# rpng/ov_plane

Hardware: AMD Instinct MI355X
Metric: MSCKF+plane update-step features/sec at 30 clones (higher is better)
Workload: dtype f64

## Files before the change

ov_plane_amd/csrc/k_chol2.h:

```cpp
#pragma once
#include <hip/hip_runtime.h>

namespace ovp {

struct Chol2Job {
  const double* A;
  int n, ld;
  int add_identity;
  int mode;
  const int* sel;
  int sel_xor;
  size_t sel_stride;
  const double* brow;
  int* flag;
  const double* floor_scale;
  double piv_floor;
  double* Lpack;
  double* Ldense;
  int ldo;
  double* z_out;
  double* y_out;
  double* piv_out;
  double* Dinv_out;
  const int* skip_cond;
  long long* stamps;
  int dbg;
  int split_h;
  double* xbuf;
  unsigned* xflag;
  unsigned xseq;
  int flip;
  double* boost;
  int boost_n;
  double boost_rel;
};

struct PlaneSolve {
  double* scal;
  unsigned* range_done;
  unsigned seq;
  double thr;
  int rows_live, rows_u, n_involved;
  int force;
  double noise_scale;
  double tol_strict, tol_loose;
  double* res_out;
  double* xzz;
  double* xy;
  unsigned* xsync;
  const double* L0;
  int ld0;
  int n_full;
  double* dx_out;
  double* dx_last;
  int* cur;
  const int* feat_list;
  int n_feat_local;
  unsigned char* feat_used;
  double *clone_R, *clone_p;
  const int* clone_id;
  int n_clones;
  double* cal;
  int calib_id, intr_id;
  double* cp;
  const int* plane_sid;
  int n_planes;
  int n_slam;
  const int* slam_id;
  double* slam_p;
  int emit, seq_plane;
  double *Lpack, *Dinv;
  int* cond;
};

}

extern "C" {
int ovp_chol2_max_n(void);
int ovp_chol2_stamps_compiled(void);
hipError_t ovp_launch_max_diag(const double* A, int n, int ld, double* out, hipStream_t stream);
hipError_t ovp_launch_chol2_packed(const double* A, double* Dinv, double* Lpack, int n, int ld, int* flag, int add_identity,
                                   const int* cond, hipStream_t stream);
hipError_t ovp_launch_chol2(const ovp::Chol2Job* j0, const ovp::Chol2Job* j1, const ovp::PlaneSolve* ps, hipStream_t stream);
}
```

ov_plane_amd/csrc/k_chol2.hip:

```cpp
#include "k_tile_body.h"
#include "k_dpp.h"
#include "k_chol2.h"
#include <cstring>

namespace ovp {

static constexpr int C2_TS = 18;
static constexpr int C2_TSZ = 16 * C2_TS;
static constexpr int C2_WAVES = 12;
static constexpr int C2_EW = 4;
static constexpr int C2_TW = C2_WAVES - C2_EW;

typedef double dbl2_t __attribute__((ext_vector_type(2)));

template <bool HAS_FLOOR, bool WRITE_PIV, bool WRITE_D>
__device__ __forceinline__ bool fused_elim16(double (&d)[16], double (&p)[16], dbl2_t* __restrict__ pvw, const double floor,
                                             dbl2_t* __restrict__ pw, dbl2_t* __restrict__ dw, const int r) {
  double piv = bcast_row<0>(d[0]), piv_prev = 0.0;
  sfor<16>([&](auto cc) {
    constexpr int c = decltype(cc)::value;
    double y0 = __builtin_amdgcn_rsq(piv);
    if constexpr (HAS_FLOOR) y0 = (piv >= floor) ? y0 : 0.0;
    const double hy = (0.5 * piv) * y0;
    const double ly = d[c] * y0, py = p[c] * y0;
    const double e = fma(-hy, y0, 0.5);
    const double l = fma(ly, e, ly);
    const double q = fma(py, e, py);
    double nl;
    asm("v_fma_f64 %0, -%1, %2, -%1\n\ts_nop 1" : "=v"(nl) : "v"(ly), "v"(e));
    d[c] = l;
    p[c] = q;
    if constexpr (WRITE_PIV && (c & 1) == 1) pvw[c >> 1] = dbl2_t{piv_prev, piv};
    piv_prev = piv;
    if constexpr (c + 1 < 16) {
      fmac_bcast<c + 1>(d[c + 1], nl, l);
      piv = bcast_row<c + 1>(d[c + 1]);
      fmac_bcast<c + 1>(p[c + 1], nl, q);
      sfor<14 - c>([&](auto jc) {
        constexpr int j = c + 2 + decltype(jc)::value;
        fmac_bcast<j>(d[j], nl, l);
        fmac_bcast<j>(p[j], nl, q);
      });
    }
    if constexpr ((c & 1) == 1) pw[c >> 1] = dbl2_t{p[c - 1], p[c]};
    if constexpr (WRITE_D && (c & 1) == 1) dw[c >> 1] = dbl2_t{(c - 1 <= r) ? d[c - 1] : 0.0, (c <= r) ? d[c] : 0.0};
  });
  return HAS_FLOOR ? false : !(piv > 0.0);
}

__device__ __forceinline__ double4_t c2_mfma_xyT(const double* X, const double* Y, double4_t acc, int off) {
  const dbl2_t* xp = reinterpret_cast<const dbl2_t*>(reinterpret_cast<const char*>(X) + off);
  const dbl2_t* yp = reinterpret_cast<const dbl2_t*>(reinterpret_cast<const char*>(Y) + off);
  dbl2_t x0 = xp[0], y0 = yp[0], x1 = xp[1], y1 = yp[1];
  asm volatile("" : "+v"(x0), "+v"(y0), "+v"(x1), "+v"(y1));
  acc = __builtin_amdgcn_mfma_f64_16x16x4f64(x0[0], y0[0], acc, 0, 0, 1);
  acc = __builtin_amdgcn_mfma_f64_16x16x4f64(x0[1], y0[1], acc, 0, 0, 1);
  acc = __builtin_amdgcn_mfma_f64_16x16x4f64(x1[0], y1[0], acc, 0, 0, 1);
  acc = __builtin_amdgcn_mfma_f64_16x16x4f64(x1[1], y1[1], acc, 0, 0, 1);
  return acc;
}

template <int NH>
__device__ __forceinline__ void c2_last_update(double* Dbuf, double* Dupd, double* Lim, const double* pbp, int k, int i0, int g, int r,
                                               bool skip) {
  const double* Pk = pbp + k * C2_TSZ;
  const dbl2_t* yp = reinterpret_cast<const dbl2_t*>(Pk + r * C2_TS + 4 * g);
  const dbl2_t y0 = yp[0], y1 = yp[1];
  double4_t acc[NH + 1];
  dbl2_t x0[NH + 1], x1[NH + 1];
#pragma unroll
  for (int t = 0; t < NH; ++t) {
    const double* im = Lim + (i0 + C2_EW * t) * C2_TSZ;
#pragma unroll
    for (int v = 0; v < 4; ++v) acc[t][v] = im[(g + 4 * v) * C2_TS + r];
    const dbl2_t* xp = reinterpret_cast<const dbl2_t*>(pbp + (i0 + C2_EW * t) * C2_TSZ + r * C2_TS + 4 * g);
    x0[t] = xp[0];
    x1[t] = xp[1];
  }
#pragma unroll
  for (int v = 0; v < 4; ++v) acc[NH][v] = Dbuf[(g + 4 * v) * C2_TS + r];
  x0[NH] = y0;
  x1[NH] = y1;
  if (!skip) {
    constexpr int NS = NH <= 1 ? NH + 1 : 1;
    constexpr int S0 = NH + 1 - NS;
    double4_t acc2[NS];
#pragma unroll
    for (int t = 0; t < NS; ++t) acc2[t] = double4_t{0.0, 0.0, 0.0, 0.0};
#pragma unroll
    for (int t = 0; t <= NH; ++t) acc[t] = __builtin_amdgcn_mfma_f64_16x16x4f64(x0[t][0], y0[0], acc[t], 0, 0, 1);
#pragma unroll
    for (int t = 0; t < NS; ++t) acc2[t] = __builtin_amdgcn_mfma_f64_16x16x4f64(x1[S0 + t][0], y1[0], acc2[t], 0, 0, 1);
#pragma unroll
    for (int t = 0; t <= NH; ++t) acc[t] = __builtin_amdgcn_mfma_f64_16x16x4f64(x0[t][1], y0[1], acc[t], 0, 0, 1);
#pragma unroll
    for (int t = 0; t < NS; ++t) acc2[t] = __builtin_amdgcn_mfma_f64_16x16x4f64(x1[S0 + t][1], y1[1], acc2[t], 0, 0, 1);
#pragma unroll
    for (int t = 0; t < S0; ++t) acc[t] = __builtin_amdgcn_mfma_f64_16x16x4f64(x1[t][0], y1[0], acc[t], 0, 0, 1);
#pragma unroll
    for (int t = 0; t < S0; ++t) acc[t] = __builtin_amdgcn_mfma_f64_16x16x4f64(x1[t][1], y1[1], acc[t], 0, 0, 1);
#pragma unroll
    for (int t = 0; t < NS; ++t) acc[S0 + t] = acc[S0 + t] + acc2[t];
  }
#pragma unroll
  for (int t = 0; t < NH; ++t) {
    double* im = Lim + (i0 + C2_EW * t) * C2_TSZ;
#pragma unroll
    for (int v = 0; v < 4; ++v) im[(g + 4 * v) * C2_TS + r] = acc[t][v];
  }
#pragma unroll
  for (int v = 0; v < 4; ++v) Dupd[(g + 4 * v) * C2_TS + r] = acc[NH][v];
}

__device__ __forceinline__ void c2_store_through_sys(double* p, dbl2_t v) {
  asm volatile("global_store_dwordx4 %0, %1, off sc0 sc1\n\ts_nop 1" ::"v"(p), "v"(v) : "memory");
}
__device__ __forceinline__ void c2_load2_through_sys(const double* p0, const double* p1, dbl2_t& v0, dbl2_t& v1) {
  asm volatile(
      "global_load_dwordx4 %0, %2, off sc0 sc1\n\t"
      "global_load_dwordx4 %1, %3, off sc0 sc1\n\t"
      "s_waitcnt vmcnt(0)"
      : "=&v"(v0), "=&v"(v1)
      : "v"(p0), "v"(p1)
      : "memory");
}

#define C2_WSYNC()                                           \
  do {                                                       \
    __builtin_amdgcn_fence(__ATOMIC_RELEASE, "workgroup");   \
    __builtin_amdgcn_wave_barrier();                         \
    __builtin_amdgcn_fence(__ATOMIC_ACQUIRE, "workgroup");   \
  } while (0)

static constexpr int C2_SPIN_LIMIT = 1 << 22;
__device__ __forceinline__ void c2_wait_ge(int* ctr, int target, int* tmo) {
  int spins = 0;
  while (__hip_atomic_load(ctr, __ATOMIC_RELAXED, __HIP_MEMORY_SCOPE_WORKGROUP) < target) {
    asm volatile("s_nop 7");
    if (__builtin_expect(++spins > C2_SPIN_LIMIT, 0)) {
      __hip_atomic_store(tmo, 1, __ATOMIC_RELAXED, __HIP_MEMORY_SCOPE_WORKGROUP);
      break;
    }
  }
  __builtin_amdgcn_fence(__ATOMIC_ACQUIRE, "workgroup");
}
__device__ __forceinline__ void c2_signal(int* ctr, int lane) {
  const unsigned a = (unsigned)(size_t)(__attribute__((address_space(3))) int*)ctr;
  asm volatile("" ::: "memory");
  if (lane == 0) asm volatile("ds_add_u32 %0, %1" ::"v"(a), "v"(1) : "memory");
  asm volatile("" ::: "memory");
}

template <int MAXSLOT, class F>
__device__ __forceinline__ void slot_range(int lo, int hi, F&& f) {
  if (lo > hi) return;
#define C2_CASE(S)                                                        \
  case S:                                                                 \
    if constexpr (S < MAXSLOT) f(std::integral_constant<int, S>{});       \
    if (hi <= S) break;                                                   \
    [[fallthrough]];
  switch (lo) {
    C2_CASE(0) C2_CASE(1) C2_CASE(2) C2_CASE(3) C2_CASE(4) C2_CASE(5) C2_CASE(6) C2_CASE(7) C2_CASE(8) C2_CASE(9) C2_CASE(10)
// ... 513 lines not shown
    for (int e = lane; e < C2_TSZ; e += 64) SD[(nt - 1) * C2_TSZ + e] = 0.0;
  if (wave == 2 || wave == 3)
    for (int e = (wave - 2) * 64 + lane; e < nt * C2_TW * 16; e += 128) SL[e] = 0.0;
  BS_STAMP(nt, 4);
  __syncthreads();
  BS_STAMP(nt, 5);
  if constexpr (ROLE == 0) {
  if (wave == 0) {
    const int r = lc;
    double y = k_hi < nt ? S.ybuf[16 * k_hi + r] : 0.0;
    double sd[16], di[16];
    auto load_sd = [&](int k) {
      const double* sblk = SD + (k >= 0 ? k : 0) * C2_TSZ + r;
#pragma unroll
      for (int c = 0; c < 16; ++c) sd[c] = sblk[c * C2_TS];
    };
    auto load_di = [&](int k) {
      const double* dblk = S.Dsave + (k >= 0 ? k : 0) * C2_TSZ + r;
#pragma unroll
      for (int c = 0; c < 16; ++c) di[c] = dblk[c * C2_TS];
    };
    load_sd(k_hi - 1);
    load_di(k_hi - 1);
    for (int k = k_hi - 1; k >= k_lo; --k) {
      BS_STAMP(k, 4);
      static_assert(C2_TW == 8, "eight partial vectors");
      const int kc = k <= nt - 3 ? k : 0;
      const double* sl = SL + ((size_t)kc * C2_TW) * 16 + r;
      int got = __hip_atomic_load(cnt_s + kc, __ATOMIC_RELAXED, __HIP_MEMORY_SCOPE_WORKGROUP);
      asm volatile("" ::: "memory");
      double p0 = sl[0], p1 = sl[16], p2 = sl[32], p3 = sl[48], p4 = sl[64], p5 = sl[80], p6 = sl[96], p7 = sl[112];
      double v = S.zbuf[16 * k + r];
      double t0 = 0.0, t1 = 0.0, t2 = 0.0, t3 = 0.0;
      fmac_bcast_nop<0>(t0, y, sd[0]);
      fmac_bcast_nop<1>(t1, y, sd[1]);
      fmac_bcast_nop<2>(t2, y, sd[2]);
      fmac_bcast_nop<3>(t3, y, sd[3]);
      fmac_bcast<4>(t0, y, sd[4]);
      fmac_bcast<5>(t1, y, sd[5]);
      fmac_bcast<6>(t2, y, sd[6]);
      fmac_bcast<7>(t3, y, sd[7]);
      fmac_bcast<8>(t0, y, sd[8]);
      fmac_bcast<9>(t1, y, sd[9]);
      fmac_bcast<10>(t2, y, sd[10]);
      fmac_bcast<11>(t3, y, sd[11]);
      fmac_bcast<12>(t0, y, sd[12]);
      fmac_bcast<13>(t1, y, sd[13]);
      fmac_bcast<14>(t2, y, sd[14]);
      fmac_bcast<15>(t3, y, sd[15]);
      double tsum = (t0 + t1) + (t2 + t3);
      asm volatile("" : "+v"(tsum));
      load_sd(k - 1);
      BS_STAMP(k, 5);
      if (k <= nt - 3) {
        const int need = (nt - k - 2 < C2_TW) ? nt - k - 2 : C2_TW;
        int spins = 0;
        while (got < need) {
          asm volatile("s_nop 7");
          if (__builtin_expect(++spins > C2_SPIN_LIMIT, 0)) {
            __hip_atomic_store(S.cnt + 6, 1, __ATOMIC_RELAXED, __HIP_MEMORY_SCOPE_WORKGROUP);
            break;
          }
          got = __hip_atomic_load(cnt_s + k, __ATOMIC_RELAXED, __HIP_MEMORY_SCOPE_WORKGROUP);
          asm volatile("" ::: "memory");
          p0 = sl[0], p1 = sl[16], p2 = sl[32], p3 = sl[48], p4 = sl[64], p5 = sl[80], p6 = sl[96], p7 = sl[112];
          asm volatile("" : "+v"(p0), "+v"(p1), "+v"(p2), "+v"(p3), "+v"(p4), "+v"(p5), "+v"(p6), "+v"(p7));
        }
        BS_STAMP(k, 6);
        v -= ((p0 + p1) + (p2 + p3)) + ((p4 + p5) + (p6 + p7));
      }
      v -= tsum;
      if (16 * k + r >= n) v = 0.0;
      double y0 = 0.0, y1 = 0.0, y2 = 0.0, y3 = 0.0;
      fmac_bcast_nop<0>(y0, v, di[0]);
      fmac_bcast_nop<1>(y1, v, di[1]);
      fmac_bcast_nop<2>(y2, v, di[2]);
      fmac_bcast_nop<3>(y3, v, di[3]);
      fmac_bcast<4>(y0, v, di[4]);
      fmac_bcast<5>(y1, v, di[5]);
      fmac_bcast<6>(y2, v, di[6]);
      fmac_bcast<7>(y3, v, di[7]);
      fmac_bcast<8>(y0, v, di[8]);
      fmac_bcast<9>(y1, v, di[9]);
      fmac_bcast<10>(y2, v, di[10]);
      fmac_bcast<11>(y3, v, di[11]);
      fmac_bcast<12>(y0, v, di[12]);
      fmac_bcast<13>(y1, v, di[13]);
      fmac_bcast<14>(y2, v, di[14]);
      fmac_bcast<15>(y3, v, di[15]);
      y = (y0 + y1) + (y2 + y3);
      if (16 * k + r >= n) y = 0.0;
      if (lane < 16) S.ybuf[16 * k + r] = y;
      c2_signal(cnt_y, lane);
      load_di(k - 1);
      BS_STAMP(k, 7);
    }
  }
  } else {
    const int tw = wave - C2_EW;
    int cur = nt;
    int pub = nt - k_hi;
    double part = 0.0;
    bool any = false;
    auto flush_to = [&](int jnew) {
      if (any && cur <= nt - 3) {
        const double pv = rows_sum_f64(part);
        if (lane < 16) SL[((size_t)cur * C2_TW + tw) * 16 + lane] = pv;
        c2_signal(cnt_s + cur, lane);
      }
      cur = jnew;
      part = 0.0;
      any = false;
    };
    sfor<MAXSLOT>([&](auto sc) {
      constexpr int s = MAXSLOT - 1 - decltype(sc)::value;
      const int i = ti[s], j = tj[s];
      if (i >= 0 && i < nt) {
        if (j != cur) flush_to(j);
        if (i >= j + 2) {
          if (pub < nt - i) {
            c2_wait_ge(cnt_y, nt - i, S.cnt + 6);
            pub = nt - i;
          }
#pragma unroll
          for (int v = 0; v < 4; ++v) part = fma(tile[s][v], S.ybuf[16 * i + lr + 4 * v], part);
          any = true;
        }
      }
    });
    flush_to(-1);
  }
  __syncthreads();
}

__device__ __forceinline__ void c2_pack_tile(double* __restrict__ Lpack, const double4_t& t, int i, int j, int n, int lr, int lc,
                                             int n_layout = 0) {
  const int ntn = ((n_layout > 0 ? n_layout : n) + 15) >> 4;
  const int tidx = j * ntn - (j * (j - 1)) / 2 + (i - j);
  double* pk = Lpack + (size_t)tidx * 256;
#pragma unroll
  for (int v = 0; v < 4; ++v) {
    const int row = lr + 4 * v, col = lc;
    const int gr = 16 * i + row, gc = 16 * j + col;
    double x = t[v];
    if (gr >= n || gc >= n) x = (gr == gc) ? 1.0 : 0.0;
    if (i == j && col > row) x = 0.0;
    pk[col * 16 + row] = x;
  }
}

static constexpr size_t C2_PS_KERNARG_OFFSET = (2 * sizeof(Chol2Job) + alignof(PlaneSolve) - 1) / alignof(PlaneSolve) * alignof(PlaneSolve);
static_assert(sizeof(Chol2Job) % alignof(Chol2Job) == 0 && alignof(Chol2Job) == 8 && alignof(PlaneSolve) == 8, "kernel-argument layout");

struct Chol2Shared {
  int bad, ok;
  double zz;
};

template <int MAXSLOT, int ROLE, bool SPLIT>
__device__ __forceinline__ void chol2_body(const Chol2Job& J0_, const PlaneSolve& ps, double* lds, Chol2Shared& sh, const int joff) {
  typedef const Chol2Job __attribute__((address_space(4))) Chol2JobK;
  typedef const char __attribute__((address_space(4))) KernargByte;
  Chol2JobK& Jf = *(Chol2JobK*)((KernargByte*)__builtin_amdgcn_kernarg_segment_ptr() + joff);
  const int n = Jf.n;
  const int nb = Jf.brow ? n + 1 : n;
  const int nt = (nb + 15) >> 4;
  const Chol2Lds S = chol2_carve(lds, nt);
  constexpr int NS = ROLE == 1 ? MAXSLOT : 1;
  if (Jf.skip_cond && Jf.skip_cond[0] != 0 && Jf.skip_cond[0] == Jf.skip_cond[1]) return;
  double4_t tile[NS];
  int ti[NS], tj[NS];
  int bad = 0;
  int& sh_bad = sh.bad;
  int& sh_ok = sh.ok;
  double& sh_zz = sh.zz;
  if (threadIdx.x == 0) sh_bad = 0;
  const int part = (SPLIT && Jf.mode == 1 && Jf.split_h > 0) ? (blockIdx.x == 2 ? 1 : 0) : -1;
  const int c_lo = part == 1 ? Jf.split_h : 0, c_hi = part == 0 ? Jf.split_h : nt;
#if C2_STAMPS_ON
  Chol2Job Jl = J0_;
  if (part == 1 && Jl.stamps) Jl.stamps += 16 * 32;
  const Chol2Job& J = Jl;
  chol2_factor<NS, ROLE, SPLIT, Chol2Job>(J, S, tile, ti, tj, bad, c_lo, c_hi);
#else
  chol2_factor<NS, ROLE, SPLIT, Chol2JobK>(Jf, S, tile, ti, tj, bad, c_lo, c_hi);
#endif
  const int tid = threadIdx.x, lane = tid & 63;
  const int wave = __builtin_amdgcn_readfirstlane(tid >> 6);
  const int lr = lane >> 4, lc = lane & 15;
  if (bad && lane == 0) atomicOr(&sh_bad, 1);
  __syncthreads();
  if (tid == 0 && S.cnt[6]) atomicOr(&sh_bad, 2);
  __syncthreads();
  bad = sh_bad;
  typedef const PlaneSolve __attribute__((address_space(4))) PlaneSolveK;
  PlaneSolveK* pk = (PlaneSolveK*)((KernargByte*)__builtin_amdgcn_kernarg_segment_ptr() + C2_PS_KERNARG_OFFSET);
  Chol2JobK* jk = (Chol2JobK*)((KernargByte*)__builtin_amdgcn_kernarg_segment_ptr() + joff);
  asm volatile("" : "+s"(pk), "+s"(jk));
  PlaneSolveK& pq = *pk;
  Chol2JobK& jq = *jk;
  if (bad && tid == 0 && jq.flag) atomicOr(jq.flag, bad);

  if (jq.mode == 0) {
    if (jq.z_out)
      for (int i = tid; i < n; i += C2_WAVES * 64) jq.z_out[i] = S.zbuf[i];
    if (jq.y_out) {
      chol2_backsolve<NS, ROLE>(S, n, (n + 15) >> 4, tile, ti, tj, jq.stamps);
      for (int i = tid; i < n; i += C2_WAVES * 64) jq.y_out[i] = S.ybuf[i];
    }
    if constexpr (ROLE == 1) {
    sfor<MAXSLOT>([&](auto sc) {
      constexpr int s = decltype(sc)::value;
      if (ti[s] >= 0) {
        if (jq.Ldense) {
#pragma unroll
          for (int v = 0; v < 4; ++v) {
            const int rr = 16 * ti[s] + lr + 4 * v, cc = 16 * tj[s] + lc;
            if (rr < nb && cc < nb) {
              const int ro = jq.flip ? n - 1 - rr : rr, rz = jq.flip ? n - 1 - cc : cc;
              jq.Ldense[(size_t)ro * jq.ldo + cc] = (cc <= rr) ? tile[s][v] : 0.0;
              if (ti[s] != tj[s]) jq.Ldense[(size_t)rz * jq.ldo + rr] = 0.0;
            }
          }
        }
        if (jq.Lpack && 16 * ti[s] < n && 16 * tj[s] < n) c2_pack_tile(jq.Lpack, tile[s], ti[s], tj[s], n, lr, lc);
      }
    });
    }
    if (jq.piv_out)
      for (int i = tid; i < n; i += C2_WAVES * 64) jq.piv_out[i] = S.pivs[i];
    if (jq.Dinv_out) {
      const int ntn = (n + 15) >> 4;
      if constexpr (ROLE == 0)
        if (!jq.y_out) c2_invert_diag_blocks(S, 0, ntn, wave, lr, lc);
      __syncthreads();
      if constexpr (ROLE == 0) {
        for (int e = tid; e < ntn * 256; e += C2_EW * 64) {
          const int k = e >> 8, i = (e >> 4) & 15, c = e & 15;
          const int gr = 16 * k + i, gc = 16 * k + c;
          jq.Dinv_out[e] = (gr < n && gc < n) ? S.Dsave[k * C2_TSZ + i * C2_TS + c] : (i == c ? 1.0 : 0.0);
        }
      }
    }
    return;
  }

  if (jq.mode == 2) {
    if (wave == 0) {
      double pr = 0.0;
      for (int i = lane; i < n; i += 64) pr = fma(S.zbuf[i], S.zbuf[i], pr);
      pr = wave_sum(pr);
      int first = 0x7fffffff, n_strict = 0;
      for (int i = lane; i < pq.n_involved; i += 64) {
        if (S.pivs[i] < pq.tol_strict) {
          ++n_strict;
          first = i < first ? i : first;
        }
      }
#pragma unroll
      for (int m = 32; m >= 1; m >>= 1) {
        n_strict += __shfl_xor(n_strict, m);
        const int o = __shfl_xor(first, m);
        first = o < first ? o : first;
      }
      int n_loose = 0;
      for (int i = lane; i < pq.n_involved; i += 64) {
        const double pv = S.pivs[i];
        if (i > first && !(pv < pq.tol_strict) && pv < pq.tol_loose) ++n_loose;
      }
#pragma unroll
      for (int m = 32; m >= 1; m >>= 1) n_loose += __shfl_xor(n_loose, m);
      if (lane == 0) {
        const int ndeg = n_strict + n_loose;
        pq.scal[1] = pr;
        pq.scal[2] = (double)ndeg;
        __threadfence();
        __hip_atomic_store(pq.range_done, pq.seq, __ATOMIC_RELEASE, __HIP_MEMORY_SCOPE_AGENT);
      }
    }
    return;
  }

#define M1_STAMP(i) C2_STAMP(nt + 1, i)
  M1_STAMP(0);
  if (wave == 0) {
    double zz = 0.0;
    for (int i = lane; i < n; i += 64) zz = fma(S.zbuf[i], S.zbuf[i], zz);
    zz = wave_sum(zz);
    if (lane == 0 && part == 0) {
      pq.xzz[0] = zz;
      pq.xzz[1] = (double)bad;
      __hip_atomic_store(pq.xsync, pq.seq, __ATOMIC_RELEASE, __HIP_MEMORY_SCOPE_AGENT);
      int spins = 0;
      unsigned v = 0u;
      bool timed_out = false;
      while (((v = __hip_atomic_load(pq.xsync + 1, __ATOMIC_ACQUIRE, __HIP_MEMORY_SCOPE_AGENT)) >> 1) != (pq.seq & 0x7fffffffu)) {
        __builtin_amdgcn_s_sleep(2);
        if (++spins > (1 << 19)) {
          timed_out = true;
          break;
        }
      }
      if (timed_out && jq.flag) atomicOr(jq.flag, 2);
      sh_zz = zz;
      sh_ok = (!timed_out && (v & 1u)) ? 1 : 0;
    } else if (lane == 0) {
      int spins = 0;
      bool timed_out = false;
      if (part == 1) {
        while (__hip_atomic_load(pq.xsync, __ATOMIC_ACQUIRE, __HIP_MEMORY_SCOPE_AGENT) != pq.seq) {
          __builtin_amdgcn_s_sleep(1);
          if (++spins > (1 << 19)) {
            timed_out = true;
            break;
          }
        }
        zz += pq.xzz[0];
        bad |= (int)pq.xzz[1];
        spins = 0;
      }
      while (__hip_atomic_load(pq.range_done, __ATOMIC_ACQUIRE, __HIP_MEMORY_SCOPE_AGENT) != pq.seq) {
        __builtin_amdgcn_s_sleep(2);
        if (++spins > (1 << 18)) {
          timed_out = true;
          break;
        }
      }
      if (timed_out && jq.flag) atomicOr(jq.flag, 2);
      const double rr = pq.scal[0], pr = pq.scal[1], ndeg = pq.scal[2];
      const double rank = (double)pq.n_involved - ndeg;
      const double noise_rows = fmax((double)pq.rows_u - rank, 0.0);
      const double denom = (double)pq.rows_live - rank;
      const double frac = denom > 0.5 ? fmin(noise_rows / denom, 1.0) : 1.0;
      const double chi2 = (pr - zz) + pq.noise_scale * frac * fmax(rr - pr, 0.0);
      const int upstream = jq.flag ? __hip_atomic_load(jq.flag, __ATOMIC_RELAXED, __HIP_MEMORY_SCOPE_AGENT) : 0;
      const bool fact_ok = (bad == 0) && !timed_out && upstream == 0;
      const bool ok = fact_ok && (pq.force == 0 ? false : (pq.force == 1 ? true : (chi2 <= pq.thr)));
      pq.res_out[0] = chi2;
      pq.res_out[1] = ok ? 1.0 : 0.0;
      pq.res_out[2] = ndeg;
      pq.res_out[3] = pr;
      sh_zz = zz;
      sh_ok = ok ? 1 : 0;
      if (part == 1 && !ok)
        __hip_atomic_store(pq.xsync + 1, (pq.seq & 0x7fffffffu) << 1, __ATOMIC_RELEASE, __HIP_MEMORY_SCOPE_AGENT);
    }
  }
  __syncthreads();
  if (!sh_ok) return;
  M1_STAMP(1);

  const int ntn = (n + 15) >> 4;
  const int h_bs = part >= 0 ? (jq.split_h < ntn ? jq.split_h : ntn) : 0;
  if (part == 0)
    for (int i = 16 * h_bs + tid; i < 16 * ntn; i += C2_WAVES * 64) S.ybuf[i] = pq.xy[i];
  chol2_backsolve<NS, ROLE>(S, n, ntn, tile, ti, tj, nullptr, part == 0 ? h_bs : ntn, part == 1 ? h_bs : 0);
  M1_STAMP(2);
  if (part == 1) {
    for (int i = 16 * h_bs + tid; i < 16 * ntn; i += C2_WAVES * 64) pq.xy[i] = S.ybuf[i];
    __syncthreads();
    if (tid == 0) {
      const bool fine = S.cnt[6] == 0;
      if (!fine) {
        if (jq.flag) atomicOr(jq.flag, 2);
        pq.res_out[1] = 0.0;
      }
      __hip_atomic_store(pq.xsync + 1, ((pq.seq & 0x7fffffffu) << 1) | (fine ? 1u : 0u), __ATOMIC_RELEASE, __HIP_MEMORY_SCOPE_AGENT);
    }
    if (pq.cond && pq.emit && S.cnt[6] == 0) {
      if constexpr (ROLE == 1) {
        sfor<MAXSLOT>([&](auto sc) {
          constexpr int s = decltype(sc)::value;
          if (ti[s] >= 0 && 16 * ti[s] < n && 16 * tj[s] < n) c2_pack_tile(pq.Lpack, tile[s], ti[s], tj[s], n, lr, lc, pq.n_full);
        });
      } else {
        for (int e = 256 * h_bs + tid; e < ntn * 256; e += C2_EW * 64) {
          const int k = e >> 8, i = (e >> 4) & 15, c = e & 15;
          const int gr = 16 * k + i, gc = 16 * k + c;
          pq.Dinv[e] = (gr < n && gc < n) ? S.Dsave[k * C2_TSZ + i * C2_TS + c] : (i == c ? 1.0 : 0.0);
        }
      }
    }
    return;
  }
  const int nfull = pq.n_full > n ? pq.n_full : n;
  double* dxs = nfull > n ? S.PB : S.zbuf;
  __syncthreads();
  if (S.cnt[6]) {
    if (tid == 0) {
      if (jq.flag) atomicOr(jq.flag, 2);
      pq.res_out[1] = 0.0;
    }
    return;
  }
  {
    const int wv = tid >> 6, ln = tid & 63;
    dbl2_t yp[3];
#pragma unroll
    for (int k = 0; k < 3; ++k) {
      const int c0 = 2 * (ln + 64 * k);
      yp[k][0] = c0 < n ? S.ybuf[c0] : 0.0;
      yp[k][1] = c0 + 1 < n ? S.ybuf[c0 + 1] : 0.0;
    }
    auto batch = [&](auto jlo_c, auto cnt_c, auto k_c) {
      constexpr int JLO = decltype(jlo_c)::value, CNT = decltype(cnt_c)::value, K = decltype(k_c)::value;
      constexpr int NP = CNT <= 2 ? 2 : (CNT <= 4 ? 4 : (CNT <= 8 ? 8 : 16));
      if (12 * JLO >= nfull) return;
      dbl2_t v[CNT][K];
#pragma unroll
      for (int j = 0; j < CNT; ++j) {
        const int row = wv + 12 * (JLO + j);
        const int lastc = row < n ? row : n - 1;
        const int npair = (lastc + 2) >> 1;
        const dbl2_t* lrow = reinterpret_cast<const dbl2_t*>(pq.L0 + (size_t)row * pq.ld0);
#pragma unroll
        for (int k = 0; k < K; ++k) {
          const int q = ln + 64 * k;
          v[j][k] = (row < nfull && q < npair) ? lrow[q] : dbl2_t{0.0, 0.0};
        }
      }
      double part[NP];
#pragma unroll
      for (int j = 0; j < NP; ++j) part[j] = 0.0;
#pragma unroll
      for (int j = 0; j < CNT; ++j) {
        const int row = wv + 12 * (JLO + j);
        const int lastc = row < n ? row : n - 1;
        double sa = 0.0;
#pragma unroll
        for (int k = 0; k < K; ++k) {
          const int c0 = 2 * (ln + 64 * k);
          sa = fma(v[j][k][0], yp[k][0], sa);
          sa = fma(c0 + 1 <= lastc ? v[j][k][1] : 0.0, yp[k][1], sa);
        }
        part[j] = sa;
      }
      const double tot = wave_transpose_reduce<NP>(part);
      const int jo = ln / (64 / NP);
      const int row = wv + 12 * (JLO + jo);
      if ((ln % (64 / NP)) == 0 && jo < CNT && row < nfull) dxs[row] = tot;
    };
    batch(std::integral_constant<int, 0>{}, std::integral_constant<int, 8>{}, std::integral_constant<int, 1>{});
    batch(std::integral_constant<int, 8>{}, std::integral_constant<int, 2>{}, std::integral_constant<int, 1>{});
    batch(std::integral_constant<int, 10>{}, std::integral_constant<int, 4>{}, std::integral_constant<int, 2>{});
    batch(std::integral_constant<int, 14>{}, std::integral_constant<int, 4>{}, std::integral_constant<int, 2>{});
    batch(std::integral_constant<int, 18>{}, std::integral_constant<int, 3>{}, std::integral_constant<int, 2>{});
    batch(std::integral_constant<int, 21>{}, std::integral_constant<int, 3>{}, std::integral_constant<int, 3>{});
  }
  __syncthreads();
  M1_STAMP(3);
  for (int i = tid; i < nfull; i += C2_WAVES * 64) {
    pq.dx_out[i] = dxs[i];
    pq.dx_last[i] = dxs[i];
  }
  if (tid == 0) *pq.cur ^= 1;
  for (int i = tid; i < pq.n_feat_local; i += C2_WAVES * 64) pq.feat_used[pq.feat_list[i]] = 1;
  auto rot_update = [&](double* R, const double* dth) {
    double qx = 0.5 * dth[0], qy = 0.5 * dth[1], qz = 0.5 * dth[2], qw = 1.0;
    const double nn = 1.0 / sqrt(qx * qx + qy * qy + qz * qz + qw * qw);
    qx *= nn;
    qy *= nn;
    qz *= nn;
    qw *= nn;
    const double a = 2.0 * qw * qw - 1.0;
    double D[9];
    D[0] = a + 2.0 * qx * qx;
    D[1] = 2.0 * qw * qz + 2.0 * qx * qy;
    D[2] = -2.0 * qw * qy + 2.0 * qx * qz;
    D[3] = -2.0 * qw * qz + 2.0 * qy * qx;
    D[4] = a + 2.0 * qy * qy;
    D[5] = 2.0 * qw * qx + 2.0 * qy * qz;
    D[6] = 2.0 * qw * qy + 2.0 * qz * qx;
    D[7] = -2.0 * qw * qx + 2.0 * qz * qy;
    D[8] = a + 2.0 * qz * qz;
    double O[9];
    for (int i = 0; i < 3; ++i)
      for (int j = 0; j < 3; ++j) O[3 * i + j] = D[3 * i] * R[j] + D[3 * i + 1] * R[3 + j] + D[3 * i + 2] * R[6 + j];
    for (int i = 0; i < 9; ++i) R[i] = O[i];
  };
  if (tid < pq.n_clones) {
    const int id = pq.clone_id[tid];
    rot_update(pq.clone_R + 9 * tid, dxs + id);
    for (int k = 0; k < 3; ++k) pq.clone_p[3 * tid + k] += dxs[id + 3 + k];
  } else if (tid == pq.n_clones) {
    if (pq.calib_id >= 0) {
      rot_update(pq.cal, dxs + pq.calib_id);
      for (int k = 0; k < 3; ++k) pq.cal[9 + k] += dxs[pq.calib_id + 3 + k];
    }
    if (pq.intr_id >= 0)
      for (int k = 0; k < 8; ++k) pq.cal[12 + k] += dxs[pq.intr_id + k];
  } else if (tid > pq.n_clones && tid <= pq.n_clones + pq.n_planes) {
    const int pl = tid - pq.n_clones - 1;
    if (pq.plane_sid[pl] >= 0)
      for (int k = 0; k < 3; ++k) pq.cp[3 * pl + k] += dxs[pq.plane_sid[pl] + k];
  }
  for (int q = tid; q < pq.n_slam; q += C2_WAVES * 64)
    for (int k = 0; k < 3; ++k) pq.slam_p[3 * q + k] += dxs[pq.slam_id[q] + k];
  M1_STAMP(4);
  if (pq.cond) {
    if (tid == 0) pq.cond[1] = pq.seq_plane;
    if (pq.emit) {
      if constexpr (ROLE == 1) {
        sfor<MAXSLOT>([&](auto sc) {
          constexpr int s = decltype(sc)::value;
          if (ti[s] >= 0 && 16 * ti[s] < n && 16 * tj[s] < n) c2_pack_tile(pq.Lpack, tile[s], ti[s], tj[s], n, lr, lc, pq.n_full);
        });
      } else {
        for (int e = tid; e < (part == 0 ? h_bs : ntn) * 256; e += C2_EW * 64) {
          const int k = e >> 8, i = (e >> 4) & 15, c = e & 15;
          const int gr = 16 * k + i, gc = 16 * k + c;
          pq.Dinv[e] = (gr < n && gc < n) ? S.Dsave[k * C2_TSZ + i * C2_TS + c] : (i == c ? 1.0 : 0.0);
        }
        if (tid == 0) pq.cond[0] = pq.seq_plane;
      }
    }
  }
}

template <int MAXSLOT, bool SPLIT>
__global__ __launch_bounds__(C2_WAVES * 64) void k_chol2(const Chol2Job J0, const Chol2Job J1, const PlaneSolve ps) {
  extern __shared__ __attribute__((aligned(16))) double lds[];
  __shared__ Chol2Shared sh;
  const Chol2Job& J = blockIdx.x == 1 ? J1 : J0;
  const int wave = __builtin_amdgcn_readfirstlane((int)threadIdx.x >> 6);
  const int joff = blockIdx.x == 1 ? (int)sizeof(Chol2Job) : 0;
  if (wave < C2_EW) chol2_body<MAXSLOT, 0, SPLIT>(J, ps, lds, sh, joff);
  else chol2_body<MAXSLOT, 1, SPLIT>(J, ps, lds, sh, joff);
}

__global__ __launch_bounds__(256) void k_max_diag(const double* __restrict__ A, int n, int ld, double* __restrict__ out) {
  __shared__ double red[256];
  double m = 0.0;
  for (int i = threadIdx.x; i < n; i += 256) m = fmax(m, A[(size_t)i * ld + i]);
  red[threadIdx.x] = m;
  __syncthreads();
  for (int s = 128; s > 0; s >>= 1) {
    if ((int)threadIdx.x < s) red[threadIdx.x] = fmax(red[threadIdx.x], red[threadIdx.x + s]);
    __syncthreads();
  }
  if (threadIdx.x == 0) out[0] = red[0];
}

}

extern "C" {

hipError_t ovp_launch_max_diag(const double* A, int n, int ld, double* out, hipStream_t stream) {
  hipLaunchKernelGGL(ovp::k_max_diag, dim3(1), dim3(256), 0, stream, A, n, ld, out);
  return hipGetLastError();
}

int ovp_chol2_max_n(void) { return 16 * 18 - 1; }

hipError_t ovp_launch_chol2_packed(const double* A, double* Dinv, double* Lpack, int n, int ld, int* flag, int add_identity,
                                   const int* cond, hipStream_t stream) {
  ovp::Chol2Job j;
  memset(&j, 0, sizeof(j));
  j.A = A;
  j.n = n;
  j.ld = ld;
  j.add_identity = add_identity;
  j.mode = 0;
  j.flag = flag;
  j.Lpack = Lpack;
  j.Dinv_out = Dinv;
  j.skip_cond = cond;
  return ovp_launch_chol2(&j, nullptr, nullptr, stream);
}

int ovp_chol2_stamps_compiled(void) { return C2_STAMPS_ON; }

hipError_t ovp_launch_chol2(const ovp::Chol2Job* j0, const ovp::Chol2Job* j1, const ovp::PlaneSolve* ps, hipStream_t stream) {
  using namespace ovp;
  auto ntof = [](const Chol2Job* j) { return ((j->brow ? j->n + 1 : j->n) + 15) / 16; };
  int nt = ntof(j0);
  int tiles = nt * (nt + 1) / 2;
  if (j0->split_h > 0) {
    const int h = j0->split_h;
    if (!j1 || !ps || j0->mode != 1 || h >= nt || !j0->xbuf || !j0->xflag || !ps->xzz || !ps->xy || !ps->xsync) return hipErrorInvalidValue;
    const int ta = h * nt - (h * (h - 1)) / 2;
    tiles = ta > tiles - ta ? ta : tiles - ta;
  }
  if (j1) {
    const int nt1 = ntof(j1);
    if (nt1 * (nt1 + 1) / 2 > tiles) tiles = nt1 * (nt1 + 1) / 2;
    if (nt1 > nt) nt = nt1;
  }
  const int slots = (tiles + C2_TW - 1) / C2_TW;
  const size_t shmem = (size_t)chol2_lds_doubles(nt) * sizeof(double);
  Chol2Job dummy = *j0;
  PlaneSolve psd = PlaneSolve();
  const Chol2Job& b = j1 ? *j1 : dummy;
  const PlaneSolve& p = ps ? *ps : psd;
  const dim3 grid(j0->split_h > 0 ? 3 : (j1 ? 2 : 1)), block(C2_WAVES * 64);
  static unsigned long long attr_mask = 0;
  if (ovp_lds_attr_needed(&attr_mask)) {
    (void)hipFuncSetAttribute((const void*)k_chol2<10, false>, hipFuncAttributeMaxDynamicSharedMemorySize, 160 * 1024);
    (void)hipFuncSetAttribute((const void*)k_chol2<15, false>, hipFuncAttributeMaxDynamicSharedMemorySize, 160 * 1024);
    (void)hipFuncSetAttribute((const void*)k_chol2<17, false>, hipFuncAttributeMaxDynamicSharedMemorySize, 160 * 1024);
    (void)hipFuncSetAttribute((const void*)k_chol2<20, false>, hipFuncAttributeMaxDynamicSharedMemorySize, 160 * 1024);
    (void)hipFuncSetAttribute((const void*)k_chol2<22, false>, hipFuncAttributeMaxDynamicSharedMemorySize, 160 * 1024);
    (void)hipFuncSetAttribute((const void*)k_chol2<13, true>, hipFuncAttributeMaxDynamicSharedMemorySize, 160 * 1024);
    (void)hipFuncSetAttribute((const void*)k_chol2<16, true>, hipFuncAttributeMaxDynamicSharedMemorySize, 160 * 1024);
    (void)hipFuncSetAttribute((const void*)k_chol2<22, true>, hipFuncAttributeMaxDynamicSharedMemorySize, 160 * 1024);
    (void)hipGetLastError();
    ovp_lds_attr_done(&attr_mask);
  }
  if (j0->split_h > 0) {
    if (slots <= 13)
      hipLaunchKernelGGL((k_chol2<13, true>), grid, block, shmem, stream, *j0, b, p);
    else if (slots <= 16)
      hipLaunchKernelGGL((k_chol2<16, true>), grid, block, shmem, stream, *j0, b, p);
    else if (slots <= 22)
      hipLaunchKernelGGL((k_chol2<22, true>), grid, block, shmem, stream, *j0, b, p);
    else
      return hipErrorInvalidValue;
    return hipGetLastError();
  }
  if (slots <= 10)
    hipLaunchKernelGGL((k_chol2<10, false>), grid, block, shmem, stream, *j0, b, p);
  else if (slots <= 15)
    hipLaunchKernelGGL((k_chol2<15, false>), grid, block, shmem, stream, *j0, b, p);
  else if (slots <= 17)
    hipLaunchKernelGGL((k_chol2<17, false>), grid, block, shmem, stream, *j0, b, p);
  else if (slots <= 20)
    hipLaunchKernelGGL((k_chol2<20, false>), grid, block, shmem, stream, *j0, b, p);
  else if (slots <= 22)
    hipLaunchKernelGGL((k_chol2<22, false>), grid, block, shmem, stream, *j0, b, p);
  else
    return hipErrorInvalidValue;
  return hipGetLastError();
}
}
```

ov_plane_amd/csrc/ovp_api_ctx.hip:

```cpp
#include "ovp_ctx.h"

static double gammap_reg(double a, double x) {
  if (x <= 0) return 0.0;
  const double gln = lgamma(a);
  if (x < a + 1.0) {
    double ap = a, sum = 1.0 / a, del = sum;
    for (int n = 0; n < 100000; ++n) {
      ap += 1.0;
      del *= x / ap;
      sum += del;
      if (fabs(del) < fabs(sum) * 1e-17) break;
    }
    return sum * exp(-x + a * log(x) - gln);
  }
  double b = x + 1.0 - a, c = 1.0 / 1e-300, d = 1.0 / b, h = d;
  for (int i = 1; i < 100000; ++i) {
    const double an = -i * (i - a);
    b += 2.0;
    d = an * d + b;
    if (fabs(d) < 1e-300) d = 1e-300;
    c = b + an / c;
    if (fabs(c) < 1e-300) c = 1e-300;
    d = 1.0 / d;
    const double del = d * c;
// ... 32 lines not shown
  switch (code) {
    case 0: return "ok";
    case OVP_E_ARG: return "bad argument";
    case OVP_E_CAPACITY: return "capacity exceeded";
    case OVP_E_NOTSPD: return "matrix not positive definite";
    case OVP_E_NEGDIAG: return "negative covariance diagonal";
    case OVP_E_NODEVICE: return "no usable HIP device";
    case OVP_E_STATE: return "call order violated";
    case OVP_E_TIMEOUT: return "device-side hand-over timed out (workgroups of the plane solve not co-resident)";
    case OVP_E_RCCL: return "RCCL not loadable or a collective call failed";
    case OVP_E_PEER: return "sharded update: the build of another rank failed (errors are collective)";
    default: return code > 0 ? hipGetErrorString((hipError_t)code) : "unknown";
  }
}


extern "C" int ovp_ctx_create(int device, int n_state_max, int n_clones_max, int n_feats_max, void* stream,
                              ovp_ctx** out) {
  if (!out || n_state_max < 1 || n_clones_max < 1 || n_clones_max > OVP_MAX_CLONES || n_feats_max < 1) return OVP_E_ARG;
  int ndev = 0;
  if (hipGetDeviceCount(&ndev) != hipSuccess || ndev <= device) return OVP_E_NODEVICE;
  HIPCHK(hipSetDevice(device));
  hipDeviceProp_t prop;
  HIPCHK(hipGetDeviceProperties(&prop, device));
  if (strncmp(prop.gcnArchName, "gfx950", 6) != 0) return OVP_E_NODEVICE;
  ovp_ctx* c = new ovp_ctx();
  c->device = device;
  if (stream) {
    c->stream = (hipStream_t)stream;
  } else {
    HIPCHK(hipStreamCreateWithFlags(&c->stream, hipStreamNonBlocking));
    c->own_stream = true;
  }
  HIPCHK(hipStreamCreateWithFlags(&c->stream2, hipStreamNonBlocking));
  HIPCHK(hipEventCreateWithFlags(&c->ev_fork, hipEventDisableTiming));
  HIPCHK(hipEventCreateWithFlags(&c->ev_join, hipEventDisableTiming));
  for (int i = 0; i < 6; ++i) HIPCHK(hipEventCreate(&c->ev_t[i]));
  HIPCHK(hipEventCreate(&c->ev_k0));
  HIPCHK(hipEventCreate(&c->ev_k1));
  c->n_max = n_state_max;
  c->c_max = n_clones_max;
  c->f_max = n_feats_max;
  c->ld = round_up(n_state_max, 16);
  c->ldg = round_up(n_state_max + 4, 16);
  if (c->ldg > OVP_LDG_CAP) return OVP_E_CAPACITY;
  const size_t nn = (size_t)(c->n_max + 1) * c->ld;
  HIPCHK(dalloc(&c->P, nn));
  HIPCHK(dalloc(&c->P_tmp, nn));
  HIPCHK(dalloc(&c->Ab, nn + 8));
  HIPCHK(dalloc(&c->L, nn));
  HIPCHK(dalloc(&c->W1, nn));
  HIPCHK(dalloc(&c->T, nn));
  HIPCHK(dalloc(&c->Lt, nn));
  HIPCHK(dalloc(&c->Y, nn));
  c->res_bytes = 16 + sizeof(double) * ((size_t)c->n_max + n_feats_max) + (size_t)n_feats_max;
  HIPCHK(hipMalloc((void**)&c->res_block, c->res_bytes));
  HIPCHK(hipMemset(c->res_block, 0, c->res_bytes));
  c->flags = (int*)c->res_block;
  c->dx = (double*)((char*)c->res_block + 16);
  c->chi2 = c->dx + c->n_max;
  c->accept = (unsigned char*)(c->chi2 + n_feats_max);
  {
    auto al = [](size_t v) { return (v + 63) & ~(size_t)63; };
    size_t o = 0;
    c->so_R = o;
    o = al(o + sizeof(double) * 9 * n_clones_max);
    c->so_Rf = o;
    o = al(o + sizeof(double) * 9 * n_clones_max);
    c->so_p = o;
    o = al(o + sizeof(double) * 3 * n_clones_max);
    c->so_pf = o;
    o = al(o + sizeof(double) * 3 * n_clones_max);
    c->so_cal = o;
    o = al(o + sizeof(double) * 32);
    c->so_id = o;
    o = al(o + sizeof(int) * n_clones_max);
    c->so_cm = o;
    o = al(o + sizeof(ovp::ColMap) * c->n_max);
    c->state_bytes = o;
    HIPCHK(hipMalloc(&c->state_block, o));
    HIPCHK(hipMemset(c->state_block, 0, o));
    HIPCHK(hipHostMalloc(&c->h_state_stage, o, hipHostMallocDefault));
    char* b = (char*)c->state_block;
    c->clone_R = (double*)(b + c->so_R);
    c->clone_R_fej = (double*)(b + c->so_Rf);
    c->clone_p = (double*)(b + c->so_p);
    c->clone_p_fej = (double*)(b + c->so_pf);
    c->cal = (double*)(b + c->so_cal);
    c->clone_id = (int*)(b + c->so_id);
    c->colmap = (ovp::ColMap*)(b + c->so_cm);
    HIPCHK(hipEventCreateWithFlags(&c->ev_state, hipEventDisableTiming));
    HIPCHK(hipEventCreateWithFlags(&c->ev_batch, hipEventDisableTiming));
  }
  HIPCHK(dalloc(&c->chi2_table, (size_t)OVP_CHI2_TABLE + 1));
  {
    const size_t F = (size_t)n_feats_max, M = OVP_MAX_MEAS;
    c->batch_cap = sizeof(double) * 3 * F + sizeof(int) * F + sizeof(int) * F * M + sizeof(float) * 2 * F * M + 256;
    HIPCHK(hipMalloc(&c->batch_block, c->batch_cap));
    HIPCHK(hipHostMalloc(&c->h_batch_stage, c->batch_cap, hipHostMallocDefault));
    c->p_FinG = (double*)c->batch_block;
  }
  HIPCHK(dalloc(&c->G, (size_t)3 * n_feats_max * c->ldg));
  HIPCHK(dalloc(&c->Bscr, (size_t)n_feats_max * OVP_BSCR));
  HIPCHK(dalloc(&c->rec, (size_t)n_clones_max * n_feats_max * 2 * 21));
  c->rows_per_chunk = 128;
  c->n_chunks = (2 * n_feats_max + c->rows_per_chunk - 1) / c->rows_per_chunk;
  HIPCHK(dalloc(&c->gramS, (size_t)n_clones_max * c->n_chunks * OVP_GRAM_ELEMS));
  HIPCHK(dalloc(&c->gramR, (size_t)n_clones_max * OVP_GRAM_ELEMS));
  HIPCHK(dalloc(&c->Dinv, (size_t)(c->ld / 16 + 1) * 256));
  {
    const size_t ntm = (size_t)c->ld / 16 + 1;
    HIPCHK(dalloc(&c->Ltp, ntm * (ntm + 1) / 2 * 256));
  }
  c->n_split = (3 * n_feats_max + 63) / 64;
  if (c->n_split < 1) c->n_split = 1;
  if (c->n_split > 64) c->n_split = 64;
  {
    const int nt = c->ldg / 16;
    HIPCHK(dalloc(&c->part, (size_t)(c->n_split + 1) * (nt * (nt + 1) / 2) * 256));
  }
  HIPCHK(dalloc(&c->idbuf, (size_t)4 * c->n_max + 64));
  c->small_cap = (size_t)4 * c->n_max * 64 + (size_t)c->n_max * c->n_max;
  HIPCHK(dalloc(&c->smallbuf, c->small_cap));
  HIPCHK(hipMalloc((void**)&c->ticket, 16));
  HIPCHK(hipMemset(c->ticket, 0, 16));
  HIPCHK(hipHostMalloc((void**)&c->h_res_block, c->res_bytes + 64, hipHostMallocMapped));
  memset(c->h_res_block, 0, c->res_bytes + 64);
  HIPCHK(hipHostGetDevicePointer(&c->h_res_block_dev, c->h_res_block, 0));
  HIPCHK(hipHostMalloc((void**)&c->h_slot, sizeof(int) * (size_t)(n_feats_max + 16), hipHostMallocMapped));
  HIPCHK(hipHostGetDevicePointer((void**)&c->d_slot, c->h_slot, 0));
  c->h_seq = (volatile unsigned*)((char*)c->h_res_block + ((c->res_bytes + 15) & ~(size_t)15));
  c->h_flags = (int*)c->h_res_block;
  c->h_dx = (double*)((char*)c->h_res_block + 16);
  c->h_chi2 = c->h_dx + c->n_max;
  c->h_accept = (unsigned char*)(c->h_chi2 + n_feats_max);
  {
    std::vector<double> tab(OVP_CHI2_TABLE + 1, 0.0);
    for (int k = 1; k <= OVP_CHI2_TABLE; ++k) tab[k] = ovp_chi2_quantile_095(k);
    HIPCHK(hipMemcpy(c->chi2_table, tab.data(), sizeof(double) * tab.size(), hipMemcpyHostToDevice));
  }
  memset(&c->fp, 0, sizeof(c->fp));
  *out = c;
  return 0;
}

extern "C" int ovp_ctx_destroy(ovp_ctx* c) {
  if (!c) return OVP_E_ARG;
  hipSetDevice(c->device);
  hipStreamSynchronize(c->stream);
  hipStreamSynchronize(c->stream2);
  void* dev[] = {c->P, c->P_tmp, c->Ab, c->L, c->W1, c->T, c->Lt, c->Y, c->res_block, c->ticket, c->uvn, c->tri_ok, c->state_block, c->batch_block,
                 c->chi2_table, c->G, c->Bscr, c->rec, c->gramS, c->gramR, c->Dinv, c->Ltp, c->part, c->idbuf, c->smallbuf, c->Hd, c->Acc,
                 c->bcc, c->resd, c->pl_slam_i, c->pl_slam_d, c->sub_ids, c->sub_buf, c->pl_Tbuf, c->pl_crow, c->pl_dxlast,
                 c->pl_cur, c->pl_perm, c->pl_range_done, c->pl_used, c->pl_dstage, c->pl_xbuf, c->pl_xy, c->pl_xflag, c->pl_Asum,
                 c->pl_U, c->pl_sub_tab, c->Lkeep, c->slam_res, c->slam_hscr, c->dinit_buf, c->boost, c->boost_vec,
                 c->gen_cal, c->gen_buf, c->pl_gen_dev};
  for (void* p : dev)
    if (p) hipFree(p);
  if (c->h_res_block) hipHostFree(c->h_res_block);
  if (c->h_slot) hipHostFree(c->h_slot);
  if (c->h_state_stage) hipHostFree(c->h_state_stage);
  if (c->h_batch_stage) hipHostFree(c->h_batch_stage);
  if (c->ev_state) hipEventDestroy(c->ev_state);
  if (c->ev_batch) hipEventDestroy(c->ev_batch);
  if (c->pl_hstage) hipHostFree(c->pl_hstage);
  if (c->pl_hres) hipHostFree(c->pl_hres);
  if (c->pl_sub_htab) hipHostFree(c->pl_sub_htab);
  if (c->ev_subtab) hipEventDestroy(c->ev_subtab);
  for (hipEvent_t e : c->pl_ev) hipEventDestroy(e);
  for (hipEvent_t e : c->pl_ev_loop) hipEventDestroy(e);
  if (c->io_h) hipHostFree(c->io_h);
  if (c->io_d) hipFree(c->io_d);
  hipEventDestroy(c->ev_fork);
  hipEventDestroy(c->ev_join);
  for (int i = 0; i < 6; ++i) hipEventDestroy(c->ev_t[i]);
  hipEventDestroy(c->ev_k0);
  hipEventDestroy(c->ev_k1);
  hipStreamDestroy(c->stream2);
  if (c->own_stream) hipStreamDestroy(c->stream);
  delete c;
  return 0;
}

extern "C" int ovp_sync(ovp_ctx* c) {
  if (!c) return OVP_E_ARG;
  HIPCHK(hipStreamSynchronize(c->stream));
  return 0;
}

extern "C" int ovp_ctx_stream(ovp_ctx* c, void** stream) {
  if (!c || !stream) return OVP_E_ARG;
  *stream = (void*)c->stream;
  return 0;
}

extern "C" int ovp_cov_size(ovp_ctx* c) { return c ? c->n : OVP_E_ARG; }

extern "C" int ovp_io_arena(ovp_ctx* c, size_t bytes, void** host, void** dev);

extern "C" int ovp_cov_upload(ovp_ctx* c, const double* P_host, int n, int ld) {
  drop_kept_factor(c);
  if (!c || !P_host || n < 1 || ld < n) return OVP_E_ARG;
  if (n > c->n_max) return OVP_E_CAPACITY;
  void *ah = nullptr, *ad = nullptr;
  const size_t bytes = sizeof(double) * (size_t)n * c->ld;
  {
    const int rca = ovp_io_arena(c, bytes, &ah, &ad);
    if (rca) return rca;
  }
  for (int i = 0; i < n; ++i) {
    memcpy((double*)ah + (size_t)i * c->ld, P_host + (size_t)i * ld, sizeof(double) * n);
    if (c->ld > n) memset((double*)ah + (size_t)i * c->ld + n, 0, sizeof(double) * (c->ld - n));
  }
  HIPCHK(hipMemcpyAsync(c->P, ah, bytes, hipMemcpyHostToDevice, c->stream));
  HIPCHK(hipStreamSynchronize(c->stream));
  c->n = n;
  c->have_cov = true;
  return 0;
}
extern "C" int ovp_cov_set_device(ovp_ctx* c, const double* P_dev, int n, int ld) {
  drop_kept_factor(c);
  if (!c || !P_dev || n < 1 || ld < n) return OVP_E_ARG;
  if (n > c->n_max) return OVP_E_CAPACITY;
  HIPCHK(hipMemcpy2DAsync(c->P, sizeof(double) * c->ld, P_dev, sizeof(double) * ld, sizeof(double) * n, n,
                          hipMemcpyDeviceToDevice, c->stream));
  c->n = n;
  c->have_cov = true;
  return 0;
}
extern "C" int ovp_cov_download(ovp_ctx* c, double* P_host, int n, int ld) {
  if (!c || !P_host || n != c->n || ld < n) return OVP_E_ARG;
  void *ah = nullptr, *ad = nullptr;
  const size_t bytes = sizeof(double) * (size_t)n * c->ld;
  {
    const int rca = ovp_io_arena(c, bytes, &ah, &ad);
    if (rca) return rca;
  }
  HIPCHK(hipMemcpyAsync(ah, c->P, bytes, hipMemcpyDeviceToHost, c->stream));
  HIPCHK(hipStreamSynchronize(c->stream));
  for (int i = 0; i < n; ++i) memcpy(P_host + (size_t)i * ld, (const double*)ah + (size_t)i * c->ld, sizeof(double) * n);
  return 0;
}
extern "C" int ovp_cov_marginal(ovp_ctx* c, const int* ids, const int* sizes, int n_vars, double* out_host) {
  if (!c || !ids || !sizes || !out_host || n_vars < 1) return OVP_E_ARG;
  std::vector<int> cols;
  for (int i = 0; i < n_vars; ++i)
    for (int k = 0; k < sizes[i]; ++k) {
      if (ids[i] + k >= c->n || ids[i] < 0) return OVP_E_ARG;
      cols.push_back(ids[i] + k);
    }
  const int m = (int)cols.size();
  if (m > c->n_max || (size_t)m * m > c->small_cap) return OVP_E_CAPACITY;
  void *ah = nullptr, *ad = nullptr;
  const size_t o_out = ((sizeof(int) * (size_t)m + 63) / 64) * 64, bytes = o_out + sizeof(double) * (size_t)m * m;
  {
    const int rca = ovp_io_arena(c, bytes, &ah, &ad);
    if (rca) return rca;
  }
  memcpy(ah, cols.data(), sizeof(int) * m);
  HIPCHK(hipMemcpyAsync(ad, ah, sizeof(int) * m, hipMemcpyHostToDevice, c->stream));
  HIPCHK(ovp_launch_gather_marginal(c->P, c->ld, (const int*)ad, m, (double*)((char*)ad + o_out), c->stream));
  HIPCHK(hipMemcpyAsync((char*)ah + o_out, (char*)ad + o_out, sizeof(double) * (size_t)m * m, hipMemcpyDeviceToHost, c->stream));
  HIPCHK(hipStreamSynchronize(c->stream));
  memcpy(out_host, (char*)ah + o_out, sizeof(double) * (size_t)m * m);
  return 0;
}

void quat_2_rot(const double q[4], double R[9]) {
  const double x = q[0], y = q[1], z = q[2], w = q[3];
  const double a = 2.0 * w * w - 1.0;
  R[0] = a + 2.0 * x * x;
  R[1] = 2.0 * w * z + 2.0 * x * y;
  R[2] = -2.0 * w * y + 2.0 * x * z;
  R[3] = -2.0 * w * z + 2.0 * y * x;
  R[4] = a + 2.0 * y * y;
  R[5] = 2.0 * w * x + 2.0 * y * z;
  R[6] = 2.0 * w * y + 2.0 * z * x;
  R[7] = -2.0 * w * x + 2.0 * z * y;
  R[8] = a + 2.0 * z * z;
}

extern "C" int ovp_state_upload(ovp_ctx* c, const ovp_state_tables* st) {
  if (!c || !st || !st->clone_q || !st->clone_p || !st->clone_q_fej || !st->clone_p_fej || !st->clone_id) return OVP_E_ARG;
  if (st->n_clones < 1 || st->n_clones > c->c_max || st->n_state > c->n_max) return OVP_E_CAPACITY;
  const int C = st->n_clones;
  for (int i = 0; i < C; ++i)
    if (st->clone_id[i] < 0 || st->clone_id[i] + 6 > st->n_state) return OVP_E_ARG;
  HIPCHK(hipEventSynchronize(c->ev_state));
  char* h = (char*)c->h_state_stage;
  double* R = (double*)(h + c->so_R);
  double* Rf = (double*)(h + c->so_Rf);
  for (int i = 0; i < C; ++i) {
    quat_2_rot(st->clone_q + 4 * i, R + 9 * i);
    quat_2_rot(st->clone_q_fej + 4 * i, Rf + 9 * i);
  }
  memcpy(h + c->so_p, st->clone_p, sizeof(double) * 3 * C);
  memcpy(h + c->so_pf, st->clone_p_fej, sizeof(double) * 3 * C);
  memcpy(h + c->so_id, st->clone_id, sizeof(int) * C);
  {
    double* cal = (double*)(h + c->so_cal);
    quat_2_rot(st->calib_q, cal);
    memcpy(cal + 9, st->calib_p, sizeof(double) * 3);
    memcpy(cal + 12, st->intrinsics, sizeof(double) * 8);
  }
  ovp::ColMap* cm = (ovp::ColMap*)(h + c->so_cm);
  memset(cm, 0, sizeof(ovp::ColMap) * c->n_max);
  for (int i = 0; i < C; ++i)
// ... 192 lines not shown
extern "C" int ovp_cov_clone_jitter(ovp_ctx* c, double relative_inflation) {
  if (!c || !(relative_inflation >= 0.0) || relative_inflation > 1e-6) return OVP_E_ARG;
  c->clone_jitter = relative_inflation;
  return 0;
}

extern "C" int ovp_cov_marginalize(ovp_ctx* c, int id, int size) {
  drop_kept_factor(c);
  if (!c || size < 1 || id < 0) return OVP_E_ARG;
  if (!c->have_cov) return OVP_E_STATE;
  if (id + size > c->n) return OVP_E_ARG;
  HIPCHK(ovp_launch_cov_marginalize(c->P, c->P_tmp, c->ld, c->n, id, size, c->stream));
  double* t = c->P;
  c->P = c->P_tmp;
  c->P_tmp = t;
  c->n -= size;
  return 0;
}

extern "C" int ovp_cov_initialize_invertible(ovp_ctx* c, const double* H_R, int k, int cols, int ld, const int* col_ids,
                                             const double* H_Linv, const double* R) {
  drop_kept_factor(c);
  if (!c || !H_R || !col_ids || !H_Linv || !R || k < 1 || k > 6 || cols < 1 || ld < k) return OVP_E_ARG;
  if (!c->have_cov) return OVP_E_STATE;
  const int n = c->n;
  if (n + k > c->n_max) return OVP_E_CAPACITY;
  if (cols > c->n_max) return OVP_E_ARG;
  for (int j = 0; j < cols; ++j)
    if (col_ids[j] < 0 || col_ids[j] >= n) return OVP_E_ARG;
  std::vector<double> hr((size_t)k * cols), hi((size_t)k * k), rk((size_t)k * k);
  for (int i = 0; i < k; ++i)
    for (int a = 0; a < cols; ++a) hr[(size_t)i * cols + a] = H_R[(size_t)a * ld + i];
  for (int i = 0; i < k; ++i)
    for (int j = 0; j < k; ++j) {
      hi[(size_t)i * k + j] = H_Linv[(size_t)j * k + i];
      rk[(size_t)i * k + j] = R[(size_t)j * k + i];
    }
  double* dHR = c->smallbuf;
  double* dHi = dHR + (size_t)k * cols;
  double* dRk = dHi + 36;
  double* dMa = dRk + 36;
  if ((size_t)(dMa + (size_t)6 * n - c->smallbuf) > c->small_cap) return OVP_E_CAPACITY;
  HIPCHK(hipMemcpyAsync(dHR, hr.data(), sizeof(double) * hr.size(), hipMemcpyHostToDevice, c->stream));
  HIPCHK(hipMemcpyAsync(dHi, hi.data(), sizeof(double) * hi.size(), hipMemcpyHostToDevice, c->stream));
  HIPCHK(hipMemcpyAsync(dRk, rk.data(), sizeof(double) * rk.size(), hipMemcpyHostToDevice, c->stream));
  HIPCHK(hipMemcpyAsync(c->idbuf, col_ids, sizeof(int) * cols, hipMemcpyHostToDevice, c->stream));
  HIPCHK(ovp_launch_init_invertible(c->P, c->ld, n, c->idbuf, cols, dHR, k, dMa, dHi, dRk, c->stream));
  HIPCHK(hipStreamSynchronize(c->stream));
  c->n = n + k;
  return 0;
}

extern "C" int ovp_cov_augment_dt(ovp_ctx* c, int pose_id, int dt_id, const double dnc_dt[6]) {
  drop_kept_factor(c);
  if (!c || !dnc_dt) return OVP_E_ARG;
  if (!c->have_cov) return OVP_E_STATE;
  if (pose_id < 0 || pose_id + 6 > c->n || dt_id < 0 || dt_id >= c->n) return OVP_E_ARG;
  HIPCHK(ovp_launch_augment_dt(c->P, c->ld, c->n, pose_id, dt_id, dnc_dt, c->stream));
  return 0;
}

extern "C" int ovp_cov_initialize(ovp_ctx* c, const double* Hx_init, const double* H_up, int k, int rup, int cols, const int* col_ids,
                                  const double* H_Linv, const double* R_init, const double* res_up, double r_iso,
                                  double chi2_threshold, int do_update, int* accepted, double* chi2, double* dx_host) {
  drop_kept_factor(c);
  if (!c || !Hx_init || !col_ids || !H_Linv || !R_init || k < 1 || k > 6 || cols < 1 || rup < 0) return OVP_E_ARG;
  if (rup > 0 && (!H_up || !res_up || !(r_iso > 0.0))) return OVP_E_ARG;
  if (!c->have_cov) return OVP_E_STATE;
  const int n = c->n, n2 = n + k, ld = c->ld, m = k + rup;
  if (n2 > c->n_max || cols > c->n_max) return OVP_E_CAPACITY;
  if (rup > ovp_init_max_rows() || ovp_init_core_lds(k, rup, cols) > ovp_init_max_lds()) return OVP_E_CAPACITY;
  for (int j = 0; j < cols; ++j)
    if (col_ids[j] < 0 || col_ids[j] >= n) return OVP_E_ARG;
  hipStream_t s = c->stream;
  const bool upd = rup > 0 && do_update;
  const size_t oHt = 0, oHi = oHt + (size_t)cols * m, oRk = oHi + 36, oRes = oRk + 36, oId = oRes + rup + 8;
  const size_t bytes = oId * sizeof(double) + sizeof(int) * (size_t)cols + 64;
  const size_t res_doubles = 4 + (size_t)c->n_max + 8;
  int rc = plane2_buffers(c, 0, bytes, res_doubles * sizeof(double));
  if (rc) return rc;
  double* h = (double*)c->pl_hstage;
  double* d = (double*)c->pl_dstage;
  for (int a = 0; a < cols; ++a) {
    double* row = h + oHt + (size_t)a * m;
    for (int i = 0; i < k; ++i) row[i] = Hx_init[(size_t)a * k + i];
    for (int i = 0; i < rup; ++i) row[k + i] = H_up[(size_t)a * rup + i];
  }
  for (int i = 0; i < 36; ++i) h[oHi + i] = h[oRk + i] = 0.0;
  for (int i = 0; i < k; ++i)
    for (int j = 0; j < k; ++j) {
      h[oHi + (size_t)i * k + j] = H_Linv[(size_t)j * k + i];
      h[oRk + (size_t)i * k + j] = R_init[(size_t)j * k + i];
    }
  for (int i = 0; i < rup; ++i) h[oRes + i] = res_up[i];
  memcpy(h + oId, col_ids, sizeof(int) * cols);
  const int* did = (const int*)(d + oId);
  double* dres = c->smallbuf;
  double* dM = dres + res_doubles;
  double* dLi = dM + (size_t)n2 * m;
  double* dy = dLi + (size_t)rup * rup;
  if ((size_t)(dy + rup + 8 - c->smallbuf) > c->small_cap) return OVP_E_CAPACITY;
  HIPCHK(hipMemcpyAsync(c->pl_dstage, c->pl_hstage, bytes, hipMemcpyHostToDevice, s));
  HIPCHK(ovp_launch_init_m(c->P, ld, n, did, cols, d + oHt, m, dM, s));
  HIPCHK(ovp_launch_init_core(c->P, ld, n, did, cols, d + oHt, k, rup, dM, d + oHi, d + oRk, d + oRes, r_iso > 0.0 ? r_iso : 1.0,
                              chi2_threshold, dLi, dy, dres, s));
  double* hres = (double*)c->pl_hres;
  if (upd) {
    HIPCHK(ovp_launch_init_update(c->P, c->P_tmp, ld, n2, dM, m, k, rup, dLi, dy, dres, dres + 4, s));
  }
  {
    const int rf = ovp_fetch_to_hres(c, dres, sizeof(double) * (upd ? 4 + (size_t)n2 : 4), s);
    if (rf) return rf;
  }
  const bool ok = hres[1] > 0.5;
  if (accepted) *accepted = ok ? 1 : 0;
  if (chi2) *chi2 = hres[0];
  if (!ok) return 0;
  c->n = n2;
  if (upd) {
    double* t = c->P;
    c->P = c->P_tmp;
    c->P_tmp = t;
  }
  if (dx_host) {
    if (upd) memcpy(dx_host, hres + 4, sizeof(double) * n2);
    else memset(dx_host, 0, sizeof(double) * n2);
  }
  if (upd && hres[2] != 0.0) return OVP_E_NEGDIAG;
  return 0;
}

extern "C" long ovp_debug_read(ovp_ctx* c, const char* name, void* host, long max_bytes) {
  if (!c || !name || !host) return OVP_E_ARG;
  const size_t nn = (size_t)(c->n_max + 1) * c->ld * sizeof(double);
  const void* src = nullptr;
  size_t bytes = 0;
  if (!strcmp(name, "A") || !strcmp(name, "Ab")) { src = c->Ab; bytes = nn; }
  else if (!strcmp(name, "L")) { src = c->L; bytes = nn; }
  else if (!strcmp(name, "T")) { src = c->T; bytes = nn; }
  else if (!strcmp(name, "Lt")) { src = c->Lt; bytes = nn; }
  else if (!strcmp(name, "Y")) { src = c->Y; bytes = nn; }
  else if (!strcmp(name, "W1")) { src = c->W1; bytes = nn; }
  else if (!strcmp(name, "P")) { src = c->P; bytes = nn; }
  else if (!strcmp(name, "G")) { src = c->G; bytes = (size_t)3 * c->n_feats * c->ldg * sizeof(double); }
  else if (!strcmp(name, "rec")) { src = c->rec; bytes = (size_t)c->fp.n_clones * c->n_feats * 2 * 21 * sizeof(double); }
  else if (!strcmp(name, "plres")) { src = c->pl_res; bytes = (size_t)4 * c->pl_cap * sizeof(double); if (!src) return OVP_E_STATE; }
  else if (!strcmp(name, "An")) { src = c->pl_An; bytes = nn; if (!src) return OVP_E_STATE; }
  else if (!strcmp(name, "bn")) { src = c->pl_bn; bytes = (size_t)c->n_max * sizeof(double); if (!src) return OVP_E_STATE; }
  else if (!strcmp(name, "pl_hres_cap")) {
    if ((size_t)max_bytes < sizeof(size_t)) return OVP_E_ARG;
    memcpy(host, &c->pl_hres_cap, sizeof(size_t));
    return (long)sizeof(size_t);
  }
  else if (!strcmp(name, "cal")) { src = c->cal; bytes = 20 * sizeof(double); if (!src) return OVP_E_STATE; }
  else if (!strcmp(name, "gen_cal")) { src = c->gen_cal; bytes = (size_t)20 * c->gen_ncams * sizeof(double); if (!src) return OVP_E_STATE; }
  else if (!strcmp(name, "dinit_planes")) {
    if (!c->pl_dstage || c->dinit_nplanes < 1) return OVP_E_STATE;
    src = (const char*)c->pl_dstage + c->dinit_pltab_off;
    bytes = (size_t)8 * c->dinit_nplanes * sizeof(double);
  }
  else if (!strcmp(name, "chi2")) {
    hipStreamSynchronize(c->stream);
    bytes = (size_t)c->n_feats * sizeof(double);
    if ((long)bytes > max_bytes) bytes = (size_t)max_bytes;
    memcpy(host, c->h_chi2, bytes);
    return (int)bytes;
  }
  else if (!strncmp(name, "bench_chol", 10)) {
    ovp_dbg_tilechol_skip = atoi(name + 10);
    hipEvent_t e0, e1;
    hipEventCreate(&e0);
    hipEventCreate(&e1);
    for (int i = 0; i < 3; ++i) ovp_launch_tilechol(c->P, c->L, c->Dinv, c->Ltp, c->n, c->ld, c->flags + 3, 0, c->stream);
    hipEventRecord(e0, c->stream);
    for (int i = 0; i < 20; ++i) ovp_launch_tilechol(c->P, c->L, c->Dinv, c->Ltp, c->n, c->ld, c->flags + 3, 0, c->stream);
    hipEventRecord(e1, c->stream);
    hipEventSynchronize(e1);
    float ms = 0.f;
    hipEventElapsedTime(&ms, e0, e1);
    ovp_dbg_tilechol_skip = 0;
    *(double*)host = ms / 20.0;
    hipEventDestroy(e0);
    hipEventDestroy(e1);
    return 8;
  }
  else if (!strcmp(name, "cycles_on")) {
    if (!c->dbg_cycles && hipMalloc((void**)&c->dbg_cycles, (size_t)c->f_max * 10 * sizeof(long long)) != hipSuccess) return OVP_E_STATE;
    return 0;
  }
  else if (!strcmp(name, "cycles")) { src = c->dbg_cycles; bytes = (size_t)c->n_feats * 10 * sizeof(long long); if (!src) return OVP_E_STATE; }
  else return OVP_E_ARG;
  if ((long)bytes > max_bytes) bytes = (size_t)max_bytes;
  if (hipStreamSynchronize(c->stream) != hipSuccess) return OVP_E_STATE;
  if (hipMemcpy(host, src, bytes, hipMemcpyDeviceToHost) != hipSuccess) return OVP_E_STATE;
  return (long)bytes;
}

static double g_dbg_chol2_floor = 0.0;
extern "C" void ovp_debug_chol2_floor(double piv_floor) { g_dbg_chol2_floor = piv_floor; }

extern "C" int ovp_debug_chol2(ovp_ctx* c, const double* A_host, int n, int lda, const double* brow_host, int add_identity,
                               double* L_host, double* z_host, double* y_host, double* piv_host, int reps, float* avg_ms) {
  if (!c || !A_host || n < 1 || lda < n) return OVP_E_ARG;
  const int nb = brow_host ? n + 1 : n;
  if (nb > ovp_chol2_max_n() + 1) return OVP_E_CAPACITY;
  double *dA = nullptr, *dL = nullptr, *dv = nullptr;
  HIPCHK(dalloc(&dA, (size_t)n * n));
  HIPCHK(dalloc(&dL, (size_t)nb * nb));
  HIPCHK(dalloc(&dv, (size_t)4 * n + 16));
  HIPCHK(hipMemcpy2D(dA, sizeof(double) * n, A_host, sizeof(double) * lda, sizeof(double) * n, n, hipMemcpyHostToDevice));
  if (brow_host) HIPCHK(hipMemcpy(dv, brow_host, sizeof(double) * n, hipMemcpyHostToDevice));
  HIPCHK(hipMemset(dL, 0, sizeof(double) * (size_t)nb * nb));
  HIPCHK(hipMemsetAsync(c->flags, 0, sizeof(int) * 4, c->stream));
  ovp::Chol2Job j;
  memset(&j, 0, sizeof(j));
  j.A = dA;
  j.n = n;
  j.ld = n;
  j.add_identity = add_identity;
  j.mode = 0;
  j.brow = brow_host ? dv : nullptr;
  j.flag = c->flags;
  j.Ldense = dL;
  j.ldo = nb;
  j.z_out = brow_host ? dv + n : nullptr;
  j.y_out = brow_host ? dv + 2 * n : nullptr;
  j.piv_out = dv + 3 * n;
  j.piv_floor = g_dbg_chol2_floor;
  HIPCHK(ovp_launch_chol2(&j, nullptr, nullptr, c->stream));
  HIPCHK(hipStreamSynchronize(c->stream));
  if (getenv("OVP_C2_STAMPS")) {
    long long* st = nullptr;
    HIPCHK(hipMalloc((void**)&st, sizeof(long long) * 16 * 32));
    HIPCHK(hipMemset(st, 0, sizeof(long long) * 16 * 32));
    ovp::Chol2Job jt = j;
    jt.Ldense = nullptr;
    if (!getenv("OVP_C2_TIME_Y")) jt.y_out = nullptr;
    jt.stamps = st;
    HIPCHK(ovp_launch_chol2(&jt, nullptr, nullptr, c->stream));
    HIPCHK(hipStreamSynchronize(c->stream));
    long long h[16 * 32];
    HIPCHK(hipMemcpy(h, st, sizeof(h), hipMemcpyDeviceToHost));
    hipFree(st);
    const int nt = (nb + 15) / 16;
    fprintf(stderr, "chol2 stamps (cycles): elimination wave 0 [wait column | read+eliminate | write] ; tile wave 0 [wait panel | reload + next column | wait buffer + publish | rest]\n");
    fprintf(stderr, " tile wave 0 prologue: issue loads %lld, patch special tiles %lld, publish column 0 %lld (elimination wave 0 starts waiting at %lld after the tile wave)\n",
            h[13] - h[16 + 13], h[14] - h[13], h[15] - h[14], h[0] - h[16 + 13]);
    for (int k = 0; k < nt; ++k) {
      const long long* e = h + k * 16;
      fprintf(stderr, " k=%2d E: %6lld %6lld %6lld | T: %6lld %6lld %6lld %6lld | E step %6lld T step %6lld | on arrival: column %+lld panel %+lld trail %+lld | E start %lld T start %lld\n", k, e[1] - e[0], e[2] - e[1],
              e[3] - e[2], e[9] - e[8], e[10] - e[9], e[11] - e[10], e[12] - e[11], e[3] - e[0], e[12] - e[8], e[4] / 1000000 - 500, (e[4] / 1000) % 1000 - 500, e[4] % 1000 - 500, e[0] - h[0], e[8] - h[0]);
    }
    if (jt.y_out) {
      fprintf(stderr, "back substitution: preparation (sub-diagonal tiles to LDS, inverses of the diagonal blocks) %lld cycles + barrier %lld, chain %lld\n",
              h[nt * 16 + 4] - h[nt * 16 + 3], h[nt * 16 + 5] - h[nt * 16 + 4], h[7] - h[nt * 16 + 5]);
      fprintf(stderr, "back substitution, wave 0 per step: [first product + loads | wait for the partial sums | sum, second product, publish]\n");
      for (int k = nt - 1; k >= 0; --k) {
        const long long* e = h + k * 16;
        fprintf(stderr, " k=%2d  %6lld %6lld %6lld | step %6lld\n", k, e[5] - e[4], k <= nt - 3 ? e[6] - e[5] : 0LL,
                e[7] - (k <= nt - 3 ? e[6] : e[5]), e[7] - e[4]);
      }
    }
  }
  if (reps > 0) {
    ovp::Chol2Job jt = j;
    jt.Ldense = nullptr;
    if (!getenv("OVP_C2_TIME_Y")) jt.y_out = nullptr;
    jt.dbg = getenv("OVP_C2_DBG") ? atoi(getenv("OVP_C2_DBG")) : 0;
    HIPCHK(hipEventRecord(c->ev_t[0], c->stream));
    for (int r = 0; r < reps; ++r) HIPCHK(ovp_launch_chol2(&jt, nullptr, nullptr, c->stream));
    HIPCHK(hipEventRecord(c->ev_t[1], c->stream));
    HIPCHK(hipStreamSynchronize(c->stream));
    float ms = 0.f;
    hipEventElapsedTime(&ms, c->ev_t[0], c->ev_t[1]);
    if (avg_ms) *avg_ms = ms / reps;
  }
  if (L_host) HIPCHK(hipMemcpy(L_host, dL, sizeof(double) * (size_t)nb * nb, hipMemcpyDeviceToHost));
  if (z_host && brow_host) HIPCHK(hipMemcpy(z_host, dv + n, sizeof(double) * n, hipMemcpyDeviceToHost));
  if (y_host && brow_host) HIPCHK(hipMemcpy(y_host, dv + 2 * n, sizeof(double) * n, hipMemcpyDeviceToHost));
  if (piv_host) HIPCHK(hipMemcpy(piv_host, dv + 3 * n, sizeof(double) * n, hipMemcpyDeviceToHost));
  int fl[4];
  HIPCHK(hipMemcpy(fl, c->flags, sizeof(fl), hipMemcpyDeviceToHost));
  HIPCHK(hipMemsetAsync(c->flags, 0, sizeof(int) * 4, c->stream));
  hipFree(dA);
  hipFree(dL);
  hipFree(dv);
  return (fl[0] & 2) ? OVP_E_TIMEOUT : (fl[0] ? OVP_E_NOTSPD : 0);
}

extern "C" int ovp_last_timings(ovp_ctx* c, float* ms4) {
  if (!c || !ms4) return OVP_E_ARG;
  memcpy(ms4, c->last_ms, sizeof(float) * 4);
  return 0;
}

extern "C" int ovp_plane_kernel_timer(ovp_ctx* c, int enable, int reset, float* avg_ms, int* n_launches) {
  if (!c) return OVP_E_ARG;
  if (avg_ms) *avg_ms = c->pl_klaunches ? (float)(c->pl_ktime_ms / c->pl_klaunches) : 0.f;
  if (n_launches) *n_launches = c->pl_klaunches;
  if (reset) {
    c->pl_ktime_ms = 0.0;
    c->pl_klaunches = 0;
  }
  c->pl_ktimer = enable;
  return 0;
}
// ... 14 lines not shown
```

ov_plane_amd/csrc/ovp_api_plane.hip:

```cpp
#include "ovp_ctx.h"

static int plane_job_device(ovp_ctx* c, const ovp_update_opts* o, const ovp::FeatParams& fp, int pl, int start, int nf,
                            int in_state, int sid, double white_c, const double* Mf, int factor_dense, double thr,
                            int rows_live, int rows_u, int n_involved, int force = -1) {
  const int n = c->n, ld = c->ld, ldg = c->ldg;
  hipStream_t s = c->stream;
  ovp::PlaneParams pp;
  pp.feat_list = c->pl_featlist + start;
  pp.n_local = nf;
  pp.plane = pl;
  pp.in_state = in_state;
  pp.plane_sid = sid;
  pp.white_c = white_c;
  pp.cp = c->pl_cp;
  pp.cp_fej = c->pl_cp_fej;
  pp.cst = c->pl_cst;
  ovp::FeatParams fpl = fp;
  fpl.n = n;
  fpl.P = c->P;
  HIPCHK(ovp_launch_plane_feat(&fpl, &pp, nf, s));
  const int chunks = (2 * nf + c->rows_per_chunk - 1) / c->rows_per_chunk;
  HIPCHK(ovp_launch_struct_gram(c->rec, fp.n_clones, nf, c->rows_per_chunk, chunks, c->gramS, s));
  HIPCHK(ovp_launch_reduce_gram(c->gramS, fp.n_clones, chunks, c->gramR, s));
  int nsplit = (3 * nf + 511) / 512;
  if (nsplit < 1) nsplit = 1;
  if (nsplit > c->n_split) nsplit = c->n_split;
  HIPCHK(ovp_launch_syrk(c->G, 3 * nf, ldg, n + 4, nsplit, c->part, s));
  HIPCHK(ovp_launch_reduce_cst(c->pl_cst, nf, c->pl_cstsum, s));
  HIPCHK(ovp_launch_assemble_ext(c->gramR, fp.n_clones, c->part, nsplit, c->colmap, n, sid, c->pl_cstsum, c->pl_E, ldg, s));
  if (!in_state && c->pl_n_slam > 0)
    HIPCHK(ovp_launch_plane_slam_rows(c->pl_E, ldg, n, pl + 1, c->pl_n_slam, c->pl_slam_i, c->pl_slam_i + c->pl_slam_cap,
                                      c->pl_slam_d, c->pl_slam_d + 3 * (size_t)c->pl_slam_cap, c->pl_cp + 3 * pl,
                                      c->pl_cp_fej + 3 * pl, white_c, fp.do_fej, c->pl_cstsum, s));
  HIPCHK(ovp_launch_plane_reduce_to_state(c->pl_E, ldg, n, in_state, c->Ab, ld, c->pl_cstsum + 9, c->pl_scal, s));
  hipStream_t s2 = c->stream2;
  HIPCHK(hipEventRecord(c->ev_fork, s));
  HIPCHK(hipStreamWaitEvent(s2, c->ev_fork, 0));
  HIPCHK(ovp_launch_normalize_reg(c->Ab, ld, n, 1e-10, c->pl_An, c->pl_bn, s2));
  HIPCHK(ovp_launch_tilechol(c->pl_An, c->pl_Lr, c->pl_Dinv2, nullptr, n, ld, c->flags + 2, 0, s2));
  HIPCHK(ovp_launch_range_energy(c->pl_Lr, c->pl_Dinv2, c->pl_bn, n, ld, 1e-8, c->pl_scal, s2));
  HIPCHK(hipEventRecord(c->ev_join, s2));
  HIPCHK(ovp_launch_gemm4(0, 0, n, n, n, c->Ab, ld, Mf, ld, c->W1, ld, 0, 0, s));
  HIPCHK(ovp_launch_gemm4(1, 0, n, n, n, Mf, ld, c->W1, ld, c->T, ld, 1, 1, s));
  HIPCHK(chol_of_T(c, c->T, n, ld, 0, nullptr, s));
  HIPCHK(ovp_launch_fwdsub(c->Ltp, c->Dinv, Mf, c->Y, n, ld, factor_dense, s));
  HIPCHK(ovp_launch_dx_from_factor(c->Y, n, ld, c->Ab + (size_t)n * ld, c->dx, c->pl_scal, s));
  HIPCHK(hipStreamWaitEvent(s, c->ev_join, 0));
  HIPCHK(ovp_launch_plane_gate(c->pl_scal, c->flags, thr, rows_live, rows_u, n_involved, force, c->pl_res + 4 * pl, s));
  return 0;
}

static int plane_buffers(ovp_ctx* c, int NP) {
  const int ld = c->ld;
  if (NP > c->pl_cap || !c->pl_E) {
    void* olds[] = {c->pl_sid, c->pl_cp, c->pl_cp_fej, c->pl_res, c->pl_dx};
    for (void* p : olds)
      if (p) hipFree(p);
    const int cap = NP + 8;
    HIPCHK(dalloc(&c->pl_sid, (size_t)cap));
    HIPCHK(dalloc(&c->pl_cp, (size_t)3 * cap));
    HIPCHK(dalloc(&c->pl_cp_fej, (size_t)3 * cap));
    HIPCHK(dalloc(&c->pl_res, (size_t)4 * cap));
    HIPCHK(dalloc(&c->pl_dx, (size_t)c->n_max * cap));
    c->pl_cap = cap;
    if (!c->pl_E) {
      const size_t ne = (size_t)(c->n_max + 4) * c->ldg;
      HIPCHK(dalloc(&c->pl_featlist, (size_t)c->f_max));
      HIPCHK(dalloc(&c->pl_cst, ((size_t)c->f_max + 1) * 10));
      HIPCHK(dalloc(&c->pl_cstsum, 16));
      HIPCHK(dalloc(&c->pl_E, ne));
      HIPCHK(dalloc(&c->pl_An, (size_t)(c->n_max + 1) * ld));
      HIPCHK(dalloc(&c->pl_bn, (size_t)c->n_max));
      HIPCHK(dalloc(&c->pl_Lr, (size_t)(c->n_max + 1) * ld));
      HIPCHK(dalloc(&c->pl_Dinv2, (size_t)(ld / 16 + 1) * 256));
      HIPCHK(dalloc(&c->pl_scal, 8));
    }
  }
  return 0;
}

struct PlaneJobH { int pl, start, nf, rows_total, rows_live, rows_u, n_involved, in_state, sid, n_inv_cols, ns_pl; double thr;
                   int g_start, ng;  };

static inline int gen_cam_col(const ovp_ctx* c, int cam, int k) {
  const int id = k < 6 ? c->gen_calib_id[cam] + k : c->gen_intr_id[cam] + (k - 6);
  if (c->pl_gen_pos.empty()) return id;
  return (id >= 0 && id < (int)c->pl_gen_pos.size()) ? c->pl_gen_pos[id] : -1;
}

extern "C" int ovp_msckf_plane_update(ovp_ctx* c, const ovp_update_opts* o, const ovp_plane_batch* pb, double* dx_planes,
                                      uint8_t* plane_ok, double* plane_chi2, int* plane_dof, uint8_t* feat_used);

__global__ __launch_bounds__(1024) void k_publish_plane_results(const double* __restrict__ res, int n_res, const double* __restrict__ dx,
                                                               int n_dx, const unsigned char* __restrict__ used, int n_used,
                                                               int* __restrict__ flags, double* __restrict__ dst_res,
                                                               double* __restrict__ dst_dx, unsigned char* __restrict__ dst_used,
                                                               int* __restrict__ dst_flags, volatile unsigned* seq_host, unsigned seq) {
  const int t = threadIdx.x;
  for (int i = t; i < n_res; i += 1024) dst_res[i] = res[i];
  for (int i = t; i < n_dx; i += 1024) dst_dx[i] = dx[i];
  {
    const int w = n_used >> 3;
    const unsigned long long* us = reinterpret_cast<const unsigned long long*>(used);
    unsigned long long* ud = reinterpret_cast<unsigned long long*>(dst_used);
    for (int i = t; i < w; i += 1024) ud[i] = us[i];
    for (int i = 8 * w + t; i < n_used; i += 1024) dst_used[i] = used[i];
  }
  if (t < 4) dst_flags[t] = flags[t];
  __threadfence_system();
  __syncthreads();
  if (t == 0) *seq_host = seq;
  if (t < 4) flags[t] = 0;
}

__global__ __launch_bounds__(1024) void k_fetch_block(const unsigned char* __restrict__ src, unsigned char* __restrict__ dst, int bytes,
                                                     volatile unsigned* seq_host, unsigned seq) {
  const int w = bytes >> 3;
  const unsigned long long* s8 = reinterpret_cast<const unsigned long long*>(src);
  unsigned long long* d8 = reinterpret_cast<unsigned long long*>(dst);
  for (int i = threadIdx.x; i < w; i += 1024) d8[i] = s8[i];
  for (int i = 8 * w + threadIdx.x; i < bytes; i += 1024) dst[i] = src[i];
  __threadfence_system();
  __syncthreads();
  if (threadIdx.x == 0) *seq_host = seq;
}
int ovp_fetch_to_hres(ovp_ctx* c, const void* dsrc, size_t bytes, hipStream_t s) {
  const size_t o_seq = c->pl_hres_cap >= 64 ? (c->pl_hres_cap - 64) & ~(size_t)63 : 0;
  if (!c->pl_hres_dev || bytes > o_seq || (((size_t)dsrc) & 7) || bytes > (size_t)0x7fffffff) {
    HIPCHK(hipMemcpyAsync(c->pl_hres, dsrc, bytes, hipMemcpyDeviceToHost, s));
    HIPCHK(hipStreamSynchronize(s));
    return 0;
  }
  volatile unsigned* hseq = (volatile unsigned*)((char*)c->pl_hres + o_seq);
  *hseq = 0u;
  const unsigned seq = ++c->pl_pub_seq;
  hipLaunchKernelGGL(k_fetch_block, dim3(1), dim3(1024), 0, s, (const unsigned char*)dsrc, (unsigned char*)c->pl_hres_dev, (int)bytes,
                     (volatile unsigned*)((char*)c->pl_hres_dev + o_seq), seq);
  HIPCHK(hipGetLastError());
  const auto t0 = std::chrono::steady_clock::now();
  unsigned spins = 0;
  while (__atomic_load_n((const unsigned*)hseq, __ATOMIC_ACQUIRE) != seq) {
    if ((++spins & 0xFFFu) == 0 && std::chrono::steady_clock::now() - t0 > std::chrono::seconds(2)) {
      HIPCHK(hipStreamSynchronize(s));
      if (__atomic_load_n((const unsigned*)hseq, __ATOMIC_ACQUIRE) != seq) return OVP_E_STATE;
      break;
    }
    __builtin_ia32_pause();
  }
  return 0;
}

static int ensure_pl_used(ovp_ctx* c) {
  if (!c->pl_used) HIPCHK(hipMalloc((void**)&c->pl_used, (size_t)c->f_max + 16));
  return 0;
}

int plane2_buffers(ovp_ctx* c, int NP, size_t stage_bytes, size_t res_bytes) {
  const int ld = c->ld;
  if (!c->pl_Tbuf) {
    const size_t nn = (size_t)(c->n_max + 1) * ld;
    HIPCHK(dalloc(&c->pl_Tbuf, 2 * nn));
    HIPCHK(dalloc(&c->pl_crow, (size_t)c->n_max + 16));
    HIPCHK(dalloc(&c->pl_dxlast, (size_t)c->n_max + 16));
    HIPCHK(hipMalloc((void**)&c->pl_cur, 16));
    HIPCHK(hipMalloc((void**)&c->pl_range_done, 16));
    HIPCHK(hipMemset(c->pl_range_done, 0, 16));
    HIPCHK(dalloc(&c->pl_xbuf, (size_t)9 * 18 * 256));
    HIPCHK(dalloc(&c->pl_xy, (size_t)c->n_max + 32));
    HIPCHK(hipMalloc((void**)&c->pl_xflag, sizeof(unsigned) * 64));
    HIPCHK(hipMemset(c->pl_xflag, 0, sizeof(unsigned) * 64));
  }
  if (NP > c->pl2_cap) {
    if (c->pl_perm) hipFree(c->pl_perm);
    c->pl2_cap = NP + 8;
    HIPCHK(hipMalloc((void**)&c->pl_perm, sizeof(int) * (size_t)c->pl2_cap * c->n_max));
  }
  if (stage_bytes > c->pl_stage_cap) {
    HIPCHK(hipStreamSynchronize(c->stream));
    if (c->pl_hstage) hipHostFree(c->pl_hstage);
    if (c->pl_dstage) hipFree(c->pl_dstage);
    c->pl_stage_cap = stage_bytes + 4096;
    HIPCHK(hipHostMalloc(&c->pl_hstage, c->pl_stage_cap, hipHostMallocDefault));
    HIPCHK(hipMalloc(&c->pl_dstage, c->pl_stage_cap));
  }
  if (res_bytes > c->pl_hres_cap) {
    HIPCHK(hipStreamSynchronize(c->stream));
    if (c->pl_hres) hipHostFree(c->pl_hres);
    c->pl_hres_cap = (res_bytes + 4096 + 63) & ~(size_t)63;
    HIPCHK(hipHostMalloc(&c->pl_hres, c->pl_hres_cap, hipHostMallocMapped));
    memset(c->pl_hres, 0, c->pl_hres_cap);
    HIPCHK(hipHostGetDevicePointer(&c->pl_hres_dev, c->pl_hres, 0));
  }
  return 0;
}

struct SubTables {
  const int* d_ids = nullptr;
  const int* d_inv = nullptr;
  int* d_clone_id = nullptr;
  ovp::ColMap* d_colmap = nullptr;
  int calib_sub = -1, intr_sub = -1;
  std::vector<int> clone_sub;
};
static int sub_tables_upload(ovp_ctx* c, const ovp_update_opts* o, const std::vector<int>& ids, const std::vector<int>& pos,
                             SubTables* t, hipStream_t s) {
  const int n = c->n, C = c->fp.n_clones, ns = (int)ids.size();
  const size_t o_ids = 0, o_inv = sizeof(int) * (size_t)(c->n_max + 16), o_tab = 2 * o_inv;
  const size_t tab_bytes = sizeof(int) * (size_t)(c->c_max + 16) + sizeof(ovp::ColMap) * (size_t)c->n_max;
  const size_t blk_bytes = o_tab + tab_bytes;
  if (!c->pl_sub_tab) {
    HIPCHK(hipMalloc(&c->pl_sub_tab, blk_bytes));
    HIPCHK(hipHostMalloc(&c->pl_sub_htab, blk_bytes, hipHostMallocDefault));
  }
  if (c->ev_subtab) HIPCHK(hipEventSynchronize(c->ev_subtab));
  else HIPCHK(hipEventCreateWithFlags(&c->ev_subtab, hipEventDisableTiming));
  char* hb = (char*)c->pl_sub_htab;
  memset(hb, 0, blk_bytes);
  int* h_ids = (int*)(hb + o_ids);
  int* h_inv = (int*)(hb + o_inv);
  int* t_clone = (int*)(hb + o_tab);
  ovp::ColMap* t_cm = (ovp::ColMap*)(hb + o_tab + sizeof(int) * (size_t)(c->c_max + 16));
  memcpy(h_ids, ids.data(), sizeof(int) * (size_t)ns);
  for (int col = 0; col < n; ++col) h_inv[col] = pos[col] >= 0 ? pos[col] : 0;
  t->clone_sub.assign((size_t)C, 0);
  for (int i = 0; i < C; ++i) {
    t->clone_sub[i] = t_clone[i] = pos[c->h_clone_id[i]];
    for (int k = 0; k < 6; ++k) {
      ovp::ColMap& m = t_cm[t->clone_sub[i] + k];
      m.kind = 1;
      m.idx = i;
      m.off = k;
    }
  }
  t->calib_sub = (c->calib_id >= 0 && c->calib_id + 6 <= n && pos[c->calib_id] >= 0) ? pos[c->calib_id] : -1;
  t->intr_sub = (c->intr_id >= 0 && c->intr_id + 8 <= n && pos[c->intr_id] >= 0) ? pos[c->intr_id] : -1;
  if (t->calib_sub >= 0 && o->do_calib_camera_pose)
    for (int k = 0; k < 6; ++k) {
      t_cm[t->calib_sub + k].kind = 2;
      t_cm[t->calib_sub + k].idx = k;
    }
  if (t->intr_sub >= 0 && o->do_calib_camera_intrinsics)
    for (int k = 0; k < 8; ++k) {
      t_cm[t->intr_sub + k].kind = 2;
      t_cm[t->intr_sub + k].idx = 6 + k;
    }
  HIPCHK(hipMemcpyAsync(c->pl_sub_tab, hb, blk_bytes, hipMemcpyHostToDevice, s));
  HIPCHK(hipEventRecord(c->ev_subtab, s));
  t->d_ids = (const int*)((char*)c->pl_sub_tab + o_ids);
  t->d_inv = (const int*)((char*)c->pl_sub_tab + o_inv);
  t->d_clone_id = (int*)((char*)c->pl_sub_tab + o_tab);
  t->d_colmap = (ovp::ColMap*)((char*)c->pl_sub_tab + o_tab + sizeof(int) * (size_t)(c->c_max + 16));
  return 0;
}
struct SubSaved {
  int n, calib_id, intr_id;
  double* P;
  int* clone_id;
  ovp::ColMap* colmap;
  const int* fp_clone_id;
  std::vector<int> h_clone_id;
};
static SubSaved sub_enter(ovp_ctx* c, const SubTables& t, int ns, double* Psub) {
  SubSaved sv{c->n, c->calib_id, c->intr_id, c->P, c->clone_id, c->colmap, c->fp.clone_id, c->h_clone_id};
  c->n = ns;
  c->P = Psub;
  c->calib_id = t.calib_sub;
  c->intr_id = t.intr_sub;
  c->clone_id = t.d_clone_id;
  c->fp.clone_id = c->clone_id;
  c->colmap = t.d_colmap;
  c->h_clone_id = t.clone_sub;
  return sv;
}
static void sub_leave(ovp_ctx* c, const SubSaved& sv) {
  c->n = sv.n;
  c->P = sv.P;
  c->calib_id = sv.calib_id;
  c->intr_id = sv.intr_id;
  c->clone_id = sv.clone_id;
  c->fp.clone_id = sv.fp_clone_id;
  c->colmap = sv.colmap;
  c->h_clone_id = sv.h_clone_id;
}

static int plane_update_ordered(ovp_ctx* c, const ovp_update_opts* o, const ovp_plane_batch* pb, double* dx_planes,
                                uint8_t* plane_ok, double* plane_chi2, int* plane_dof, uint8_t* feat_used) {
  const double t_entry = host_now_ms();
  const int n = c->n, ld = c->ld, NP = pb->n_planes, C = c->fp.n_clones;
  const int n_slam = pb->n_slam > 0 ? pb->n_slam : 0;
  if (n_slam > 0 && (!pb->slam_plane || !pb->slam_state_id || !pb->slam_p || !pb->slam_p_fej)) return OVP_E_ARG;
  std::vector<int> ids, pos((size_t)n, -1);
  ids.reserve((size_t)n);
  bool bad_id = false;
  auto place = [&](int id, int sz) {
    if (id < 0 || id + sz > n) {
      bad_id = true;
      return;
    }
    for (int k = 0; k < sz; ++k)
      if (pos[id + k] < 0) {
        pos[id + k] = (int)ids.size();
        ids.push_back(id + k);
      }
  };
  for (int i = 0; i < C; ++i) place(c->h_clone_id[i], 6);
  if (o->do_calib_camera_pose) place(c->calib_id, 6);
  if (o->do_calib_camera_intrinsics) place(c->intr_id, 8);
  if (c->pl_gen_b)
    for (int k = 0; k < c->gen_ncams; ++k) {
      if (o->do_calib_camera_pose) place(c->gen_calib_id[k], 6);
      if (o->do_calib_camera_intrinsics) place(c->gen_intr_id[k], 8);
    }
  for (int q = 0; q < n_slam; ++q)
    if (pb->slam_plane[q] < 1 || pb->slam_plane[q] > NP || pb->slam_state_id[q] < 0 || pb->slam_state_id[q] + 3 > n) return OVP_E_ARG;
  c->pl_nl.assign((size_t)(NP > 0 ? NP : 1), 0);
  for (int k = 0; k < NP; ++k) {
    if (pb->plane_state_id[k] >= 0) place(pb->plane_state_id[k], 3);
    else
      for (int q = 0; q < n_slam; ++q)
        if (pb->slam_plane[q] == k + 1) place(pb->slam_state_id[q], 3);
    c->pl_nl[k] = (int)ids.size();
  }
  if (bad_id) return OVP_E_ARG;
// ... 234 lines not shown
  for (int pl = 1; pl <= NP + 1; ++pl) gbucket[pl] += gbucket[pl - 1];
  {
    std::vector<int> fill(gbucket.begin(), gbucket.end());
    for (int g = 0; g < GF; ++g)
      if (c->pl_gen_plane[g] >= 1 && c->pl_gen_plane[g] <= NP && gbp->n_meas[g] >= 2) gsorted[fill[c->pl_gen_plane[g]]++] = g;
  }
  int ng_max = 0;
  for (int pl = 0; pl < NP; ++pl) {
    PlaneJobH j;
    j.pl = pl;
    j.start = (int)featlist.size();
    j.nf = 0;
    j.rows_total = 0;
    j.rows_live = 0;
    j.sid = pb->plane_state_id[pl];
    j.in_state = j.sid >= 0;
    unsigned long long seen = 0ull;
    for (int bi = bucket_start[pl + 1]; bi < bucket_start[pl + 2]; ++bi) {
      const int f = bucket[bi];
      const int m = c->h_n_meas[f];
      if (m < 2) continue;
      if (m > OVP_MAX_MEAS_DEV) return bail(OVP_E_CAPACITY);
      featlist.push_back(f);
      j.nf++;
      j.rows_total += 3 * m - 3;
      j.rows_live += 2 * m - 2;
      for (int k = 0; k < m; ++k) seen |= 1ull << c->h_clone_idx[(size_t)f * M + k];
    }
    j.g_start = (int)glist.size();
    j.ng = 0;
    unsigned cams_seen = j.nf > 0 ? 1u : 0u;
    for (int gi = gbucket[pl + 1]; gi < gbucket[pl + 2]; ++gi) {
      const int g = gsorted[gi], m = gbp->n_meas[g];
      glist.push_back(g);
      j.ng++;
      j.rows_total += 3 * m - 3;
      j.rows_live += 2 * m - 2;
      for (int k = 0; k < m; ++k) {
        seen |= 1ull << gbp->clone_idx[(size_t)g * GM + k];
        cams_seen |= 1u << gbp->cam_idx[(size_t)g * GM + k];
      }
    }
    const int ncal_pl = j.ng > 0 ? ncal * __builtin_popcount(cams_seen) : ncal;
    int ns_pl = 0;
    if (!j.in_state)
      for (int q = 0; q < n_slam; ++q)
        if (pb->slam_plane[q] == pl + 1) ++ns_pl;
    if (ns_pl > PA_MAXQ) return bail(OVP_E_CAPACITY);
    j.ns_pl = ns_pl;
    if (j.nf + j.ng == 0 || (!j.in_state && j.nf + j.ng + ns_pl < 4)) {
      featlist.resize(j.start);
      glist.resize(j.g_start);
      continue;
    }
    j.rows_total += ns_pl;
    j.rows_live += ns_pl;
    const int c_ref = 6 * __builtin_popcountll(seen) + ncal_pl + 3 * ns_pl;
    const int rows_c = j.rows_total > c_ref ? c_ref : j.rows_total;
    j.rows_u = j.in_state ? rows_c : rows_c - 3;
    j.n_involved = c_ref + (j.in_state ? 3 : 0);
    if (!j.in_state) j.rows_total -= 3;
    if (!j.in_state) j.rows_live -= 3;
    if (j.rows_u < 1) {
      featlist.resize(j.start);
      glist.resize(j.g_start);
      continue;
    }
    if (j.ng > ng_max) ng_max = j.ng;
    j.thr = o->chi2_multiplier * ovp_chi2_quantile_095(j.rows_u);
    {
      std::vector<int> perm(n, -1);
      int pos = 0;
      std::vector<char> inv(n, 0);
      const bool cam0 = j.ng == 0 || (cams_seen & 1u);
      if (o->do_calib_camera_pose && cam0)
        for (int k = 0; k < 6; ++k) inv[c->calib_id + k] = 1;
      if (o->do_calib_camera_intrinsics && cam0)
        for (int k = 0; k < 8; ++k) inv[c->intr_id + k] = 1;
      if (j.ng > 0)
        for (int cam = 0; cam < c->gen_ncams; ++cam)
          if ((cams_seen >> cam) & 1u)
            for (int k = 0; k < 14; ++k) {
              if (!(k < 6 ? o->do_calib_camera_pose : o->do_calib_camera_intrinsics)) continue;
              const int col = gen_cam_col(c, cam, k);
              if (col < 0 || col >= n) return bail(OVP_E_ARG);
              inv[col] = 1;
            }
      if (j.in_state)
        for (int k = 0; k < 3; ++k) inv[j.sid + k] = 1;
      if (!j.in_state)
        for (int q = 0; q < n_slam; ++q)
          if (pb->slam_plane[q] == pl + 1)
            for (int k = 0; k < 3; ++k) inv[pb->slam_state_id[q] + k] = 1;
      for (int col = 0; col < n; ++col)
        if (inv[col]) perm[col] = pos++;
      for (int ci = 0; ci < (int)c->h_clone_id.size(); ++ci)
        if ((seen >> ci) & 1ull)
          for (int k = 0; k < 6; ++k) {
            const int col = c->h_clone_id[ci] + k;
            if (col >= 0 && col < n && perm[col] < 0) perm[col] = pos++;
          }
      j.n_inv_cols = pos;
      perms.insert(perms.end(), perm.begin(), perm.end());
    }
    jobs.push_back(j);
  }
  const int NJ = (int)jobs.size();
  if (NJ == 0 && any_candidate) {
    HIPCHK(join_chol());
    HIPCHK(hipMemsetAsync(c->flags, 0, sizeof(int) * 4, s));
  }
  const size_t n_int = featlist.size() + (size_t)NP + perms.size() + 2 * (size_t)n_slam;
  const size_t int_bytes = ((n_int * sizeof(int) + 15) / 16) * 16;
  const size_t n_dbl = 6 * (size_t)NP + 6 * (size_t)n_slam;
  const size_t stage_bytes = int_bytes + n_dbl * sizeof(double);
  rc = plane2_buffers(c, NP, stage_bytes, res_bytes);
  if (rc) return rc;
  int* hi = (int*)c->pl_hstage;
  double* hd = (double*)((char*)c->pl_hstage + int_bytes);
  int* di = (int*)c->pl_dstage;
  double* dd = (double*)((char*)c->pl_dstage + int_bytes);
  size_t io = 0;
  const size_t o_feat = io;
  memcpy(hi + io, featlist.data(), sizeof(int) * featlist.size());
  io += featlist.size();
  const size_t o_sid = io;
  memcpy(hi + io, pb->plane_state_id, sizeof(int) * NP);
  io += NP;
  const size_t o_perm = io;
  if (!perms.empty()) memcpy(hi + io, perms.data(), sizeof(int) * perms.size());
  io += perms.size();
  const size_t o_spl = io;
  if (n_slam) memcpy(hi + io, pb->slam_plane, sizeof(int) * n_slam);
  io += n_slam;
  const size_t o_sidx = io;
  if (n_slam) memcpy(hi + io, pb->slam_state_id, sizeof(int) * n_slam);
  io += n_slam;
  memcpy(hd, pb->cp, sizeof(double) * 3 * NP);
  memcpy(hd + 3 * NP, pb->cp_fej, sizeof(double) * 3 * NP);
  if (n_slam) {
    memcpy(hd + 6 * NP, pb->slam_p, sizeof(double) * 3 * n_slam);
    memcpy(hd + 6 * NP + 3 * n_slam, pb->slam_p_fej, sizeof(double) * 3 * n_slam);
  }
  HIPCHK(hipMemcpyAsync(c->pl_dstage, c->pl_hstage, stage_bytes, hipMemcpyHostToDevice, s));
  const int* d_feat = di + o_feat;
  const int* d_sid = di + o_sid;
  const int* d_perm = di + o_perm;
  const int* d_spl = di + o_spl;
  const int* d_sidx = di + o_sidx;
  double* d_cp = dd;
  double* d_cpfej = dd + 3 * NP;
  double* d_slam_p = dd + 6 * NP;
  double* d_slam_pfej = dd + 6 * NP + 3 * n_slam;
  ovp::PlaneGenParams gp0;
  ovp::PlaneGenCols gcols;
  memset(&gp0, 0, sizeof(gp0));
  memset(&gcols, 0xff, sizeof(gcols));
  const unsigned gen_calmask = (o->do_calib_camera_pose ? 0x3Fu : 0u) | (o->do_calib_camera_intrinsics ? (0xFFu << 6) : 0u);
  if (gbp) {
    for (int cam = 0; cam < c->gen_ncams; ++cam)
      for (int k = 0; k < 14; ++k)
        if ((gen_calmask >> k) & 1u) {
          gcols.col[cam][k] = gen_cam_col(c, cam, k);
          if (gcols.col[cam][k] < 0 || gcols.col[cam][k] >= n) return bail(OVP_E_ARG);
        }
  }
  if (gbp && !glist.empty()) {
    auto al = [](size_t v) { return (v + 63) & ~(size_t)63; };
    const size_t GFM = (size_t)GF * GM;
    const size_t o_uv = 0, o_ci = al(sizeof(float) * 2 * GFM), o_cam = al(o_ci + sizeof(int) * GFM), o_nm = al(o_cam + sizeof(int) * GFM),
                 o_p = al(o_nm + sizeof(int) * GF), o_list = al(o_p + sizeof(double) * 3 * GF), in_bytes = al(o_list + sizeof(int) * glist.size());
    const size_t mark_stride = (size_t)((n + 4 + 15) & ~15), hp_stride = (size_t)ovp::PG_ROWS * (n + 4);
    const size_t o_hp = al(sizeof(int) * mark_stride * ng_max), total = o_hp + sizeof(double) * hp_stride * ng_max;
    if (total > c->pl_gen_cap) {
      HIPCHK(hipStreamSynchronize(s));
      if (c->pl_gen_dev) HIPCHK(hipFree(c->pl_gen_dev));
      c->pl_gen_dev = nullptr;
      c->pl_gen_cap = 0;
      HIPCHK(hipMalloc(&c->pl_gen_dev, total + total / 2));
      c->pl_gen_cap = total + total / 2;
    }
    void *ah = nullptr, *ad = nullptr;
    {
      const int rca = ovp_io_arena(c, in_bytes, &ah, &ad);
      if (rca) return bail(rca);
    }
    char* h = (char*)ah;
    memcpy(h + o_uv, gbp->uv, sizeof(float) * 2 * GFM);
    memcpy(h + o_ci, gbp->clone_idx, sizeof(int) * GFM);
    memcpy(h + o_cam, gbp->cam_idx, sizeof(int) * GFM);
    memcpy(h + o_nm, gbp->n_meas, sizeof(int) * GF);
    memcpy(h + o_p, gbp->p_FinG, sizeof(double) * 3 * GF);
    memcpy(h + o_list, glist.data(), sizeof(int) * glist.size());
    HIPCHK(hipMemcpyAsync(ad, ah, in_bytes, hipMemcpyHostToDevice, s));
    char* d = (char*)ad;
    char* ds = (char*)c->pl_gen_dev;
    gp0.fp = fp;
    gp0.fp.calmask = gen_calmask;
    gp0.cam_cal = c->gen_cal;
    for (int k = 0; k < OVP_MAX_CAMERAS; ++k) gp0.cam_fisheye[k] = c->gen_fisheye[k];
    gp0.cc = gcols;
    gp0.uv = (const float*)(d + o_uv);
    gp0.clone_idx = (const int*)(d + o_ci);
    gp0.cam_idx = (const int*)(d + o_cam);
    gp0.n_meas = (const int*)(d + o_nm);
    gp0.p_FinG = (const double*)(d + o_p);
    gp0.max_meas = GM;
    gp0.list = (const int*)(d + o_list);
    gp0.mark = (int*)ds;
    gp0.mark_stride = (int)mark_stride;
    gp0.hp = (double*)(ds + o_hp);
    gp0.hp_stride = hp_stride;
  }
  const double white_c = 1.0 / o->sigma_constraint;
  double noise_scale = OVP_PLANE_NOISE_KAPPA;
  if (const char* ns_env = getenv("OVP_PL_NOISE_SCALE")) noise_scale = atof(ns_env);
  for (int jn = 0; jn < NJ; ++jn) {
    const PlaneJobH& j = jobs[jn];
    const int nk = c->pl_sub_active ? c->pl_nl[j.pl] : n;
    ovp::PlaneParams pp;
    pp.feat_list = d_feat + j.start;
    pp.n_local = j.nf;
    pp.plane = j.pl;
    pp.in_state = j.in_state;
    pp.plane_sid = j.sid;
    pp.white_c = white_c;
    pp.cp = d_cp;
    pp.cp_fej = d_cpfej;
    pp.cst = c->pl_cst;
    ovp::FeatParams fpl = fp;
    fpl.n = nk;
    fpl.P = c->P;
    int chunks = (2 * j.nf + c->rows_per_chunk - 1) / c->rows_per_chunk;
    int nsplit = 1;
    if (j.nf > 0) {
      HIPCHK(ovp_launch_plane_feat(&fpl, &pp, j.nf, s));
      HIPCHK(ovp_launch_gram_pair(c->rec, fp.n_clones, j.nf, c->rows_per_chunk, chunks, c->gramS, c->G, 3 * j.nf, c->ldg, nk + 4,
                                  c->n_split, c->part, &nsplit, s));
    } else {
      chunks = 1;
      nsplit = 0;
      HIPCHK(hipMemsetAsync(c->gramS, 0, sizeof(double) * (size_t)fp.n_clones * OVP_GRAM_ELEMS, s));
    }
    const int nt16_pl = (nk + 4 + 15) / 16, ntile_pl = nt16_pl * (nt16_pl + 1) / 2;
    if (j.ng > 0) {
      ovp::PlaneGenParams g = gp0;
      g.list = gp0.list + j.g_start;
      g.n_local = j.ng;
      g.plane = j.pl;
      g.in_state = j.in_state;
      g.plane_sid = j.sid;
      g.white_c = white_c;
      g.cp = d_cp;
      g.cp_fej = d_cpfej;
      g.n = nk;
      g.hp_stride = (size_t)ovp::PG_ROWS * (nk + 4);
      g.part_split = c->part + (size_t)nsplit * ntile_pl * 256;
      g.cst_rec = c->pl_cst + (size_t)j.nf * 10;
      HIPCHK(ovp_launch_plane_feat_gen(&g, s));
    }
    ovp::PlaneAsm pa;
    memset(&pa, 0, sizeof(pa));
    pa.gramS = c->gramS;
    pa.n_clones = fp.n_clones;
    pa.n_chunks = chunks;
    pa.part = c->part;
    pa.n_split = nsplit + (j.ng > 0 ? 1 : 0);
    pa.ntile = ntile_pl;
    pa.colmap = c->colmap;
    pa.n = nk;
    pa.plane_sid = j.sid;
    pa.in_state = j.in_state;
    pa.cst = c->pl_cst;
    pa.nf = j.nf + (j.ng > 0 ? 1 : 0);
    pa.n_slam = j.in_state ? 0 : n_slam;
    pa.plane1 = j.pl + 1;
    pa.slam_plane = d_spl;
    pa.slam_id = d_sidx;
    pa.slam_p = d_slam_p;
    pa.slam_p_fej = d_slam_pfej;
    pa.cp = d_cp + 3 * j.pl;
    pa.cp_fej = d_cpfej + 3 * j.pl;
    pa.white_c = white_c;
    pa.do_fej = fp.do_fej;
    pa.Ab = c->Ab;
    pa.lda = ld;
    pa.perm = d_perm + (size_t)jn * n;
    pa.An = c->pl_An;
    pa.ldn = ld;
    pa.bn = c->pl_bn;
    pa.eps = 1e-12;
    pa.scal = c->pl_scal;
    HIPCHK(ovp_launch_plane_assemble2(&pa, s));
    HIPCHK(join_chol());
    HIPCHK(ovp_launch_gemm4(0, 0, nk, nk, nk, c->Ab, ld, c->L, ld, c->W1, ld, 0, 0, s));
    HIPCHK(ovp_launch_plane_dT(nk, c->L, ld, c->W1, c->Ab + (size_t)nk * ld, c->pl_Tbuf, tstride, c->pl_cur, c->pl_crow, s));
    ovp::Chol2Job j0, j1;
    memset(&j0, 0, sizeof(j0));
    memset(&j1, 0, sizeof(j1));
    j0.A = c->pl_Tbuf;
    j0.sel = c->pl_cur;
    j0.sel_xor = 1;
    j0.sel_stride = tstride;
    j0.n = nk;
    j0.ld = ld;
    j0.add_identity = 1;
    j0.mode = 1;
    j0.brow = c->pl_crow;
    j0.flag = c->flags;
    j1.A = c->pl_An;
    j1.n = j.n_inv_cols;
    j1.ld = ld;
    j1.add_identity = 0;
    j1.mode = 2;
    j1.brow = c->pl_bn;
    j1.flag = c->flags + 2;
    j1.piv_floor = 1e-5;
    ovp::PlaneSolve ps;
    memset(&ps, 0, sizeof(ps));
    ps.scal = c->pl_scal;
    ps.range_done = c->pl_range_done;
    ps.seq = ++c->pl_seq;
    {
      const char* split_s = getenv("OVP_C2_SPLIT");
      const int split_env = split_s ? atoi(split_s) : -1;
      const int nb = nk + 1, ntb = (nb + 15) / 16;
      const int nst = (nb % 16 == 1) ? ntb - 1 : ntb;
      int h = ntb >= 17 ? nst / 3 : 0;
      if (split_env >= 0) h = split_env < ntb - 1 ? split_env : 0;
      if (h > 9) h = 9;
      j0.split_h = h;
      j0.xbuf = c->pl_xbuf;
      j0.xflag = c->pl_xflag;
      j0.xseq = ps.seq;
      ps.xzz = c->pl_xy;
      ps.xy = c->pl_xy + 16;
      ps.xsync = c->pl_xflag + 32;
    }
    ps.thr = j.thr;
    ps.rows_live = j.rows_live;
    ps.rows_u = j.rows_u;
    ps.n_involved = j.n_inv_cols;
    ps.force = pb->force_decision ? (int)pb->force_decision[j.pl] : -1;
    ps.noise_scale = noise_scale;
    ps.tol_strict = 1e-5;
    ps.tol_loose = 1e-5;
    ps.res_out = c->pl_res + 4 * j.pl;
    ps.L0 = c->L;
    ps.ld0 = ld;
    ps.n_full = n;
    ps.dx_out = c->pl_dx + (size_t)j.pl * n;
    ps.dx_last = c->pl_dxlast;
    ps.cur = c->pl_cur;
    const int emit_last = 4;
    ps.cond = c->pl_cur + 1;
    ps.seq_plane = jn + 1;
    ps.emit = (jn >= NJ - emit_last) ? 1 : 0;
    ps.Lpack = c->Ltp;
    ps.Dinv = c->Dinv;
    ps.feat_list = d_feat + j.start;
    ps.n_feat_local = j.nf;
    ps.feat_used = c->pl_used;
    ps.clone_R = c->clone_R;
    ps.clone_p = c->clone_p;
    ps.clone_id = c->clone_id;
    ps.n_clones = fp.n_clones;
    ps.cal = c->cal;
    ps.calib_id = o->do_calib_camera_pose ? c->calib_id : -1;
    ps.intr_id = o->do_calib_camera_intrinsics ? c->intr_id : -1;
    ps.cp = d_cp;
    ps.plane_sid = d_sid;
    ps.n_planes = NP;
    ps.n_slam = n_slam;
    ps.slam_id = d_sidx;
    ps.slam_p = d_slam_p;
    if (c->pl_ktimer == 1) {
      while ((int)c->pl_ev.size() < 2 * (jn + 1)) {
        hipEvent_t e;
        HIPCHK(hipEventCreate(&e));
        c->pl_ev.push_back(e);
      }
      HIPCHK(hipEventRecord(c->pl_ev[2 * jn], s));
    }
    static const bool pl_stamps = getenv("OVP_PL_STAMPS") != nullptr && ovp_chol2_stamps_compiled();
    static long long* d_stamps = nullptr;
    if (pl_stamps) {
      if (!d_stamps) HIPCHK(hipMalloc((void**)&d_stamps, sizeof(long long) * 2 * 16 * 32));
      j0.stamps = d_stamps;
    }
    HIPCHK(ovp_launch_chol2(&j0, &j1, &ps, s));
    if (c->pl_ktimer == 1) HIPCHK(hipEventRecord(c->pl_ev[2 * jn + 1], s));
    if (gbp)
      HIPCHK(ovp_launch_plane_gen_commit(c->pl_res + 4 * j.pl, c->pl_dx + (size_t)j.pl * n, c->gen_cal, c->gen_ncams, &gcols,
                                         gen_calmask, s));
    if (c->pl_sub_rest)
      HIPCHK(ovp_launch_plane_sub_accum(c->pl_res + 4 * j.pl, c->Ab, c->pl_Asum, c->pl_dx + (size_t)j.pl * n,
                                        c->pl_U + (size_t)j.pl * ld, nk, ld, s));
    if (pl_stamps && jn == NJ - 1) {
      long long h[2 * 16 * 32];
      HIPCHK(hipStreamSynchronize(s));
      HIPCHK(hipMemcpy(h, d_stamps, sizeof(h), hipMemcpyDeviceToHost));
      const int ntb = (nk + 1 + 15) / 16;
      const long long* e = h + (ntb + 1) * 16;
      fprintf(stderr, "[plane tail, cycles] factor %lld | gate %lld | back substitution %lld | dx = L0 y %lld | commit %lld\n",
              e[0] - h[0], e[1] - e[0], e[2] - e[1], e[3] - e[2], e[4] - e[3]);
      if (atoi(getenv("OVP_PL_STAMPS")) >= 2) {
        const long long t0 = h[0];
        for (int part = 0; part < (j0.split_h > 0 ? 2 : 1); ++part) {
          const long long* hp = h + part * 16 * 32;
          fprintf(stderr, " part %c: prologue stamps %lld %lld %lld\n", part ? 'B' : 'A', hp[13] - t0, hp[14] - t0, hp[15] - t0);
          for (int k = 0; k < ntb; ++k) {
            const long long* q = hp + k * 16;
            if (!q[0] && !q[8]) continue;
            const long long aw = q[4] - 500500500;
            const long long am = llround((double)aw / 1e6), ar = aw - am * 1000000, ap = llround((double)ar / 1e3), at = ar - ap * 1000;
            fprintf(stderr, "  k=%2d E %7lld %7lld %7lld %7lld [%3lld %3lld %3lld] | T %7lld %7lld %7lld %7lld %7lld | T7 %7lld %7lld %7lld\n", k,
                    q[0] - t0, q[1] - t0, q[2] - t0, q[3] - t0, am, ap, at, q[8] - t0, q[9] - t0, q[10] - t0, q[11] - t0, q[12] - t0,
                    q[7] - t0, q[5] - t0, q[6] - t0);
            if (k >= 2 && atoi(getenv("OVP_PL_STAMPS")) >= 3) fprintf(stderr, "        T own tiles final %7lld, column k+1 taken %7lld\n", q[13] - t0, q[14] - t0);
          }
          const long long* m = hp + (ntb + 1) * 16;
          fprintf(stderr, "  tail: factor done %lld, gate %lld, backsolve %lld, dx %lld, commit %lld\n", m[0] - t0, m[1] - t0, m[2] - t0,
                  m[3] - t0, m[4] - t0);
        }
      }
      HIPCHK(hipMemset(d_stamps, 0, sizeof(long long) * 2 * 16 * 32));
    }
  }
  bool factor_enqueued = false;
  if (NJ > 0) {
    {
      if (n <= ovp_chol2_max_n() + 1) {
        ovp::Chol2Job jt;
        memset(&jt, 0, sizeof(jt));
        jt.A = c->pl_Tbuf;
        jt.sel = c->pl_cur;
        jt.sel_xor = 0;
        jt.sel_stride = tstride;
        jt.n = n;
        jt.ld = ld;
        jt.add_identity = 1;
        jt.mode = 0;
        jt.flag = c->flags;
        jt.Lpack = c->Ltp;
        jt.Dinv_out = c->Dinv;
        jt.skip_cond = c->pl_cur + 1;
        HIPCHK(ovp_launch_chol2(&jt, nullptr, nullptr, s));
      } else {
        HIPCHK(ovp_launch_select_copy(c->T, c->pl_Tbuf, tstride, c->pl_cur, n, ld, 1, s));
        HIPCHK(chol_of_T(c, c->T, n, ld, 1, c->pl_cur + 1, s));
      }
    }
    HIPCHK(ovp_launch_fwdsub(c->Ltp, c->Dinv, c->L, c->Y, n, ld, 0, s));
    HIPCHK(ovp_launch_gemm4c(1, 0, n, n, n, c->Y, ld, c->Y, ld, c->P, ld, 0, 1, c->flags, s));
    const bool keep_factor = getenv("OVP_NO_KEPT_FACTOR") == nullptr;
    const bool want_factor = keep_factor && !c->pl_sub_rest && n <= OVP_TILECHOL_NMAX;
    if (want_factor && !c->Lkeep) HIPCHK(dalloc(&c->Lkeep, (size_t)c->n_max * ld));
    if (c->pl_scatter_dst) {
      HIPCHK(ovp_launch_unpermute_pair(c->P, c->Y, ld, c->pl_scatter_ids, n, c->pl_scatter_dst, want_factor ? c->Lkeep : nullptr, ld,
                                       c->flags, c->pl_boost_active ? c->boost_vec : nullptr, s));
      c->kept_boost = want_factor && c->pl_boost_active;
    } else if (want_factor) {
      HIPCHK(ovp_launch_factor_from_V(c->Y, ld, nullptr, n, c->Lkeep, ld, s));
    }
    factor_enqueued = want_factor;
  }
  if (c->pl_ktimer) HIPCHK(hipEventRecord(c->pl_ev_loop[1], s));
  double* hres = (double*)c->pl_hres;
  double* hdx = hres + 4 * (size_t)NP;
  unsigned char* hused = (unsigned char*)(hdx + (size_t)n * NP);
  char* hflags_pub = (char*)hused + (((size_t)F + 63) & ~(size_t)63);
  volatile unsigned* hseq = (volatile unsigned*)(hflags_pub + 64);
  *hseq = 0u;
  const unsigned seq = ++c->pl_pub_seq;
  {
    char* dbase = (char*)c->pl_hres_dev;
    auto dev_of = [&](const void* hp) { return dbase + ((const char*)hp - (const char*)c->pl_hres); };
    hipLaunchKernelGGL(k_publish_plane_results, dim3(1), dim3(1024), 0, s, c->pl_res, 4 * NP, c->pl_dx, dx_planes ? n * NP : 0, c->pl_used,
                       F, c->flags, (double*)dev_of(hres), (double*)dev_of(hdx), (unsigned char*)dev_of(hused), (int*)dev_of(hflags_pub),
                       (volatile unsigned*)dev_of((const void*)hseq), seq);
    HIPCHK(hipGetLastError());
  }
  const double t_enq = host_now_ms();
  {
    const auto t0 = std::chrono::steady_clock::now();
    unsigned spins = 0;
    while (__atomic_load_n((const unsigned*)hseq, __ATOMIC_ACQUIRE) != seq) {
      if ((++spins & 0xFFFu) == 0 && std::chrono::steady_clock::now() - t0 > std::chrono::seconds(2)) {
        HIPCHK(hipStreamSynchronize(s));
        if (__atomic_load_n((const unsigned*)hseq, __ATOMIC_ACQUIRE) != seq) return OVP_E_STATE;
        break;
      }
      __builtin_ia32_pause();
    }
    memcpy(c->h_flags, hflags_pub, sizeof(int) * 4);
  }
  {
    c->host_acc[0] += t_first - t_entry;
    c->host_acc[1] += t_enq - t_entry;
    c->host_acc[2] += host_now_ms() - t_enq;
    c->host_acc[3] += 1.0;
  }
  if (c->pl_ktimer) {
    float ms = 0.f;
    if (hipEventElapsedTime(&ms, c->pl_ev_loop[0], c->pl_ev_loop[1]) == hipSuccess) c->host_acc[7] += ms;
  }
  if (c->pl_ktimer == 1)
    for (int jn = 0; jn < NJ; ++jn) {
      float ms = 0.f;
      if (hipEventElapsedTime(&ms, c->pl_ev[2 * jn], c->pl_ev[2 * jn + 1]) == hipSuccess) {
        c->pl_ktime_ms += ms;
        c->pl_klaunches += 1;
      }
    }
  c->pl_used_valid = true;
  c->h_pl_used.assign(hused, hused + F);
  if (dx_planes) memcpy(dx_planes, hdx, sizeof(double) * (size_t)n * NP);
  if (feat_used && F) memcpy(feat_used, hused, (size_t)F);
  if (gbp) {
    c->pl_gen_used.assign((size_t)GF, 0);
    for (const PlaneJobH& j : jobs)
      if (hres[4 * j.pl + 1] > 0.5)
        for (int k = 0; k < j.ng; ++k) c->pl_gen_used[glist[j.g_start + k]] = 1;
  }
  for (const PlaneJobH& j : jobs) {
    if (plane_ok) plane_ok[j.pl] = hres[4 * j.pl + 1] > 0.5 ? 1 : 0;
    if (plane_chi2) plane_chi2[j.pl] = hres[4 * j.pl];
    if (plane_dof) plane_dof[j.pl] = j.rows_u;
// ... 225 lines not shown
```

ov_plane_amd/csrc/ovp_ctx.h:

```cpp
#pragma once
#include "ovplane_hip.h"

#include <hip/hip_runtime.h>
#include <math.h>
#include <stdio.h>
#include <stdlib.h>
#include <string.h>
#include <dlfcn.h>

#include <algorithm>
#include <chrono>
#include <vector>

#include "ovp_kernels.h"
#include "k_chol2.h"
#include "k_plane2.h"
#include "k_slam.h"
#include "k_dinit.h"
#include "k_plane_gen.h"

extern "C" int ovp_dbg_tilechol_skip;
extern "C" {
hipError_t ovp_launch_scatter_gram_add(const double* Acc, const double* bcc, int cols, const int* col_ids, double* Ab, int lda, int n,
                                       hipStream_t stream);
// ... 19 lines not shown
                                      hipStream_t stream);
hipError_t ovp_launch_propagate(double* P, int ldp, int n, int start, int phi, const int* oldcol, int nold,
                                const double* Phi, const double* Q, double* CPT, double* PCP, int* negdiag,
                                hipStream_t stream);
hipError_t ovp_launch_propagate_publish(double* P, int ldp, int n, int start, int phi, const int* oldcol, int nold, const double* Phi,
                                        const double* Q, double* CPT, double* PCP, int* negdiag, unsigned* host_dev, unsigned seq,
                                        hipStream_t stream);
hipError_t ovp_launch_augment_dt(double* P, int ldp, int n, int pose, int dt, const double* d, hipStream_t stream);
hipError_t ovp_launch_init_invertible(double* P, int ldp, int n, const int* cols, int ncols, const double* HR, int k,
                                      double* Ma, const double* Hinv, const double* Rk, hipStream_t stream);
hipError_t ovp_launch_tilechol_unless(const double* A, double* L, double* Dinv, double* Lpack, int n, int ld, int* flag,
                                      int add_identity, const int* cond, hipStream_t stream);
hipError_t ovp_launch_tilechol(const double* A, double* L, double* Dinv, double* Lpack, int n, int ld, int* flag, int add_identity,
                               hipStream_t stream);
hipError_t ovp_launch_fwdsub_lead(const double* Ltp, const double* Dinv, const double* Lmat, double* V, int n, int ld, int dense,
                                  int n_lead, hipStream_t stream);
hipError_t ovp_launch_fwdsub(const double* Lt, const double* Dinv, const double* Lmat, double* V, int n, int ld,
                             int dense, hipStream_t stream);
hipError_t ovp_launch_gemm4(int transA, int transB, int M, int N, int K, const double* A, int lda, const double* B,
                            int ldb, double* C, int ldc, int add_identity, int symmetric, hipStream_t stream);
hipError_t ovp_launch_dx_rows_boost(double* P, int n, int ldp, const double* b, double* dx, int* negdiag, unsigned* ticket,
                                    void* res_block, void* host_block, int pub_words, void* seq_host, unsigned seq,
                                    const double* boost, int boost_n, const int* cancel, hipStream_t stream);
hipError_t ovp_launch_dx_rows(const double* P, int n, int ldp, const double* b, double* dx, int* negdiag,
                              unsigned* ticket, void* res_block, void* host_block, int pub_words, void* seq_host,
                              unsigned seq,
                              hipStream_t stream);
hipError_t ovp_launch_reduce_gram(const double* gramS, int n_clones, int n_chunks, double* gramR, hipStream_t stream);
hipError_t ovp_launch_plane_feat(const ovp::FeatParams* p, const ovp::PlaneParams* pp, int n_local, hipStream_t stream);
hipError_t ovp_launch_reduce_cst(const double* cst, int nf, double* out, hipStream_t stream);
hipError_t ovp_launch_assemble_ext(const double* gramR, int n_clones, const double* part, int n_split,
                                   const ovp::ColMap* colmap, int n, int plane_sid, const double* cstsum, double* E,
                                   int lde, hipStream_t stream);
hipError_t ovp_launch_plane_reduce_to_state(const double* E, int lde, int n, int in_state, double* Ab, int lda,
                                            const double* rr_in, double* scal, hipStream_t stream);
hipError_t ovp_launch_normalize_reg(const double* Ab, int lda, int n, double eps, double* An, double* bn,
                                    hipStream_t stream);
hipError_t ovp_launch_range_energy(const double* Lr, const double* Dinv, const double* bn, int n, int ld, double tol,
                                   double* scal, hipStream_t stream);
hipError_t ovp_launch_dx_from_factor(const double* V, int n, int ld, const double* b, double* dx, double* scal,
                                     hipStream_t stream);
hipError_t ovp_launch_init_m(const double* P, int ldp, int n, const int* ids, int cols, const double* Ht, int m, double* Mall,
                             hipStream_t stream);
hipError_t ovp_launch_init_core(double* P, int ldp, int n, const int* ids, int cols, const double* Ht, int k, int rup, double* Mall,
                                const double* Hinv, const double* Rk, const double* resid, double r_iso, double thr, double* Linv,
                                double* y, double* res, hipStream_t stream);
hipError_t ovp_launch_init_update(const double* Psrc, double* Pdst, int ldp, int n2, const double* Mall, int m, int k, int rup,
                                  const double* Linv, const double* y, double* res, double* dx, hipStream_t stream);
hipError_t ovp_launch_init_m_sk(const double* skip, const double* P, int ldp, int n, const int* ids, int cols, const double* Ht, int m,
                                double* Mall, hipStream_t stream);
hipError_t ovp_launch_init_core_sk(const double* skip, double* P, int ldp, int n, const int* ids, int cols, const double* Ht, int k,
                                   int rup, double* Mall, const double* Hinv, const double* Rk, const double* resid, double r_iso,
                                   double thr, double* Linv, double* y, double* res, hipStream_t stream);
hipError_t ovp_launch_init_update_sk(const double* skip, int res_len, const double* Psrc, double* Pdst, int ldp, int n2,
                                     const double* Mall, int m, int k, int rup, const double* Linv, const double* y, double* res,
                                     double* dx, hipStream_t stream);
size_t ovp_init_core_lds(int k, int rup, int cols);
size_t ovp_init_max_lds();
int ovp_init_max_rows();
hipError_t ovp_launch_gemm4c(int transA, int transB, int M, int N, int K, const double* A, int lda, const double* B, int ldb,
                             double* C, int ldc, int add_identity, int symmetric, const int* cancel, hipStream_t stream);
hipError_t ovp_launch_plane_gate(const double* scal, const int* flags, double thr, int rows_live, int rows_u,
                                 int n_involved, int force, double* res_out, hipStream_t stream);
hipError_t ovp_launch_plane_init_augment(const double* E, int lde, int ns, const int* ids, int n, double* P, int ldp, const double* dx, double* out,
                                         hipStream_t stream);
hipError_t ovp_launch_plane_slam_rows(double* E, int lde, int n, int plane1, int n_slam, const int* slam_plane, const int* slam_id,
                                      const double* slam_p, const double* slam_p_fej, const double* cp, const double* cp_fej,
                                      double white_c, int do_fej, double* cstsum, hipStream_t stream);
hipError_t ovp_launch_plane_commit_slam(const double* res, const double* dx, int n_slam, const int* slam_id, double* slam_p,
                                        hipStream_t stream);
hipError_t ovp_launch_plane_commit(const double* res, const double* V, double* M, int n, int ld, const double* dx,
                                   double* dx_out, double* clone_R, double* clone_p, const int* clone_id, int n_clones,
                                   double* cal, int calib_id, int intr_id, double* cp, const int* plane_sid,
                                   int n_planes, hipStream_t stream);
}


static const int OVP_TILECHOL_NMAX = 288;

#define HIPCHK(x)                               \
  do {                                          \
    hipError_t _e = (x);                        \
    if (_e != hipSuccess) return (int)_e;       \
  } while (0)

static inline int round_up(int v, int m) { return ((v + m - 1) / m) * m; }

struct ovp_ctx {
  int device = 0;
  hipStream_t stream = nullptr, stream2 = nullptr;
  bool own_stream = false;
  hipEvent_t ev_fork = nullptr, ev_join = nullptr;
  hipEvent_t ev_t[6] = {nullptr, nullptr, nullptr, nullptr, nullptr, nullptr};
  int n_max = 0, c_max = 0, f_max = 0;
  int n = 0, ld = 0;
  double *P = nullptr, *P_tmp = nullptr;
  double *clone_R = nullptr, *clone_p = nullptr, *clone_R_fej = nullptr, *clone_p_fej = nullptr;
  int* clone_id = nullptr;
  double* cal = nullptr;
  ovp::ColMap* colmap = nullptr;
  double* chi2_table = nullptr;
  ovp::FeatParams fp;
  bool have_state = false, have_cov = false, have_batch = false;
  float* uv = nullptr;
  int *clone_idx = nullptr, *n_meas = nullptr;
  double* p_FinG = nullptr;
  int n_feats = 0, max_meas = 0;
  double *G = nullptr, *rec = nullptr, *chi2 = nullptr, *Bscr = nullptr;
  unsigned char* accept = nullptr;
  float* uvn = nullptr;
  unsigned char* tri_ok = nullptr;
  int ldg = 0;
  double *gramS = nullptr, *gramR = nullptr, *part = nullptr, *Dinv = nullptr, *Ltp = nullptr;
  int n_chunks = 0, rows_per_chunk = 0, n_split = 0;
  double* Ab = nullptr;
  double *L = nullptr, *W1 = nullptr, *T = nullptr, *Lt = nullptr, *Y = nullptr;
  double* dx = nullptr;
  int* flags = nullptr;
  double *Hd = nullptr, *Acc = nullptr, *bcc = nullptr, *resd = nullptr;
  std::vector<int> dense_cols;
  std::vector<double> dense_A, dense_b;
  int gen_ncams = 0;
  int gen_calib_id[OVP_MAX_CAMERAS] = {-1, -1, -1, -1}, gen_intr_id[OVP_MAX_CAMERAS] = {-1, -1, -1, -1};
  int gen_fisheye[OVP_MAX_CAMERAS] = {0, 0, 0, 0};
  double gen_cal_h[OVP_MAX_CAMERAS * 20] = {};
  double* gen_cal = nullptr;
  void* gen_buf = nullptr;
  size_t gen_cap = 0;
  void* slam_res = nullptr;
  double* slam_hscr = nullptr;
  size_t slam_res_cap = 0, slam_hscr_cap = 0;
  double* dinit_buf = nullptr;
  size_t dinit_cap = 0;
  size_t dinit_pltab_off = 0;
  int dinit_nplanes = 0;
  size_t Hd_cap = 0, res_cap = 0;
  int calib_id = -1, intr_id = -1;
  long long* dbg_cycles = nullptr;
  std::vector<int> h_n_meas, h_clone_idx;
  int *pl_featlist = nullptr, *pl_sid = nullptr;
  double *pl_cp = nullptr, *pl_cp_fej = nullptr, *pl_cst = nullptr, *pl_cstsum = nullptr, *pl_E = nullptr;
  double *pl_An = nullptr, *pl_bn = nullptr, *pl_Lr = nullptr, *pl_Dinv2 = nullptr, *pl_scal = nullptr;
  double *pl_res = nullptr, *pl_dx = nullptr;
  int pl_cap = 0;
  int *pl_slam_i = nullptr;
  double *pl_slam_d = nullptr;
  int pl_slam_cap = 0, pl_n_slam = 0;
  double *pl_Tbuf = nullptr, *pl_crow = nullptr, *pl_dxlast = nullptr;
  int *pl_cur = nullptr, *pl_perm = nullptr;
  unsigned* pl_range_done = nullptr;
  unsigned pl_seq = 0;
  int range_lo = -1, range_hi = -1;
  unsigned char* pl_used = nullptr;
  std::vector<unsigned char> h_pl_used;
  int* h_slot = nullptr;
  int* d_slot = nullptr;
  bool pl_used_valid = false;
  int pl2_cap = 0;
  void *io_h = nullptr, *io_d = nullptr;
  size_t io_cap = 0;
  double *pl_xbuf = nullptr, *pl_xy = nullptr;
  unsigned* pl_xflag = nullptr;
  double *pl_Asum = nullptr, *pl_U = nullptr;
  int pl_U_cap = 0;
  void *pl_sub_tab = nullptr, *pl_sub_htab = nullptr;
  bool pl_sub_active = false;
  bool pl_sub_rest = false;
  std::vector<int> pl_nl;
  double* pl_scatter_dst = nullptr;
  const int* pl_scatter_ids = nullptr;
  double pl_t_entry = 0.0;
  bool pl_psd = false;
  const ovp_general_batch* pl_gen_b = nullptr;
  const int* pl_gen_plane = nullptr;
  std::vector<int> pl_gen_pos;
  std::vector<unsigned char> pl_gen_used;
  void* pl_gen_dev = nullptr;
  size_t pl_gen_cap = 0;
  double* Lkeep = nullptr;
  bool have_factor = false, use_kept_factor = false;
  double clone_jitter = 0.0;
  double* boost_vec = nullptr;
  bool pl_boost_active = false, kept_boost = false;
  double* boost = nullptr;
  int point_boost_n = 0;
  int point_nl = 0;
  hipEvent_t ev_subtab = nullptr;
  void *pl_hstage = nullptr, *pl_dstage = nullptr;
  size_t pl_stage_cap = 0;
  void* pl_hres = nullptr;
  void* pl_hres_dev = nullptr;
  unsigned pl_pub_seq = 0;
  size_t pl_hres_cap = 0;
  void *state_block = nullptr, *h_state_stage = nullptr, *batch_block = nullptr, *h_batch_stage = nullptr;
  size_t state_bytes = 0, batch_cap = 0;
  size_t so_R = 0, so_Rf = 0, so_p = 0, so_pf = 0, so_cal = 0, so_id = 0, so_cm = 0;
  hipEvent_t ev_state = nullptr, ev_batch = nullptr;
  int pl_ktimer = 0;
  std::vector<hipEvent_t> pl_ev, pl_ev_loop;
  double pl_ktime_ms = 0.0;
  int pl_klaunches = 0;
  int* idbuf = nullptr;
  double* smallbuf = nullptr;
  size_t small_cap = 0;
  int* sub_ids = nullptr;
  int sub_ns = 0;
  std::vector<int> h_clone_id;
  double* sub_buf = nullptr;
  double *h_dx = nullptr, *h_chi2 = nullptr;
  unsigned char* h_accept = nullptr;
  int* h_flags = nullptr;
  void *res_block = nullptr, *h_res_block = nullptr;
  void* h_res_block_dev = nullptr;
  volatile unsigned* h_seq = nullptr;
  unsigned prop_seq = 0;
  unsigned seq = 0, pub_seq = 0;
  bool pub_pending = false;
  bool need_join = false;
  unsigned* ticket = nullptr;
  std::vector<int> h_nmeas;
  bool h_nmeas_valid = false;
  size_t res_bytes = 0;
  float last_ms[4] = {0, 0, 0, 0};
  bool timed = false;
  bool ktimer = false;
  hipEvent_t ev_k0 = nullptr, ev_k1 = nullptr;
  double ktime_ms = 0.0;
  int klaunches = 0;
  bool kpending = false;
  double host_acc[8] = {0, 0, 0, 0, 0, 0, 0, 0};
};

static inline void drop_kept_factor(ovp_ctx* c) {
  if (!c) return;
  c->have_factor = false;
  c->use_kept_factor = false;
  c->point_nl = 0;
  c->point_boost_n = 0;
  c->kept_boost = false;
  c->dense_cols.clear();
}

static inline double host_now_ms() {
  return std::chrono::duration<double, std::milli>(std::chrono::steady_clock::now().time_since_epoch()).count();
}


template <class T>
static hipError_t dalloc(T** p, size_t count) {
  return hipMalloc((void**)p, count * sizeof(T));
}

void quat_2_rot(const double q[4], double R[9]);
extern "C" int ovp_io_arena(ovp_ctx* c, size_t bytes, void** host, void** dev);
int fill_feat_params(ovp_ctx* c, const ovp_update_opts* o);
int check_general_batch(const ovp_ctx* c, const ovp_general_batch* b, bool need_p, const int* only = nullptr, bool any_length = false);
int ovp_fetch_to_hres(ovp_ctx* c, const void* dsrc, size_t bytes, hipStream_t s);
int chol_of_P(ovp_ctx* c, hipStream_t s);
hipError_t chol_of_T(ovp_ctx* c, const double* T, int n, int ld, int add_identity, const int* cond, hipStream_t s);
int set_substate(ovp_ctx* c, const std::vector<int>& ids);
int ekf_from_gram(ovp_ctx* c, bool chol_p_done_on_stream2, bool publish = false);
int ekf_sform(ovp_ctx* c);
int plane2_buffers(ovp_ctx* c, int NP, size_t stage_bytes, size_t res_bytes);
```

Baseline: 791,100.

## Offload plane dx product and state update to helper workgroups

Adds extra helper workgroups to the fused Cholesky plane-update kernel. They preload rows of the L0 matrix into LDS, wait on a flag for the back-solved y vector, compute the dx = L0·y product for their row range, and apply the clone, calibration, plane and SLAM state updates. The main workgroup now only publishes y and signals, so the serial tail after the solve is split across several workgroups. A prefetch variant that caches clone and plane state in LDS is also added. The cost is extra spin-wait synchronisation through global flags, more launched workgroups, and system-scope loads.

```diff
diff --git a/ov_plane_amd/csrc/k_chol2.h b/ov_plane_amd/csrc/k_chol2.h
--- a/ov_plane_amd/csrc/k_chol2.h
+++ b/ov_plane_amd/csrc/k_chol2.h
@@ -71,7 +71,37 @@
   int emit, seq_plane;
   double *Lpack, *Dinv;
   int* cond;
+  int n_help;
+  int help_row[5];
+  double* hy;
+  unsigned* hsync;
 };
+
+static constexpr int C2_MAX_HELP = 4;
+static constexpr int C2_HELP_OVERLAP = 8;
+static constexpr int C2_HELP_NMAX = 288;
+static constexpr int C2_HELP_HDR = 2 * C2_HELP_NMAX;
+static constexpr int C2_HELP_LDS_MAX = 150 * 1024;
+inline __host__ __device__ int c2_help_row_pairs(int row, int n) { return ((row < n ? row : n - 1) + 2) >> 1; }
+inline bool c2_help_fits(int n, int nfull, int n_clones, int n_planes, int nh, const int* rows, size_t* lds_bytes) {
+  if (nh < 1 || nh > C2_MAX_HELP || n < 1 || n > 3 * 128 || nfull < n || nfull > C2_HELP_NMAX) return false;
+  if (n_clones + n_planes + 1 > 12 * 64) return false;
+  if (rows[0] != 0 || rows[nh] != nfull) return false;
+  size_t most = 0;
+  for (int h = 0; h < nh; ++h) {
+    const int r0 = rows[h], r1 = rows[h + 1];
+    if (r0 < 0 || r1 <= r0 || r1 > nfull) return false;
+    const int rend = r1 + C2_HELP_OVERLAP < nfull ? r1 + C2_HELP_OVERLAP : nfull;
+    size_t pairs = 0;
+    for (int r = r0; r < rend; ++r) pairs += (size_t)c2_help_row_pairs(r, n);
+    const size_t need = (size_t)C2_HELP_HDR * sizeof(double) + 16 * pairs;
+    if (need > (size_t)C2_HELP_LDS_MAX) return false;
+    if (need > most) most = need;
+  }
+  if (lds_bytes) *lds_bytes = most;
+  return true;
+}
+static constexpr int C2_XFLAG_STEP = 0, C2_XFLAG_XSYNC = 32, C2_XFLAG_HSYNC = 48, C2_XFLAG_WORDS = 64;
 
 }
 
diff --git a/ov_plane_amd/csrc/k_chol2.hip b/ov_plane_amd/csrc/k_chol2.hip
--- a/ov_plane_amd/csrc/k_chol2.hip
+++ b/ov_plane_amd/csrc/k_chol2.hip
@@ -8,6 +8,7 @@
 static constexpr int C2_TS = 18;
 static constexpr int C2_TSZ = 16 * C2_TS;
 static constexpr int C2_WAVES = 12;
+static_assert(C2_WAVES * 64 == 12 * 64, "c2_help_fits (k_chol2.h) counts one thread of a workgroup per table entry");
 static constexpr int C2_EW = 4;
 static constexpr int C2_TW = C2_WAVES - C2_EW;
 
@@ -827,13 +828,236 @@
 static constexpr size_t C2_PS_KERNARG_OFFSET = (2 * sizeof(Chol2Job) + alignof(PlaneSolve) - 1) / alignof(PlaneSolve) * alignof(PlaneSolve);
 static_assert(sizeof(Chol2Job) % alignof(Chol2Job) == 0 && alignof(Chol2Job) == 8 && alignof(PlaneSolve) == 8, "kernel-argument layout");
 
+__device__ __forceinline__ void c2_rot_update(double* R, const double* dth) {
+  double qx = 0.5 * dth[0], qy = 0.5 * dth[1], qz = 0.5 * dth[2], qw = 1.0;
+  const double nn = 1.0 / sqrt(qx * qx + qy * qy + qz * qz + qw * qw);
+  qx *= nn;
+  qy *= nn;
+  qz *= nn;
+  qw *= nn;
+  const double a = 2.0 * qw * qw - 1.0;
+  double D[9];
+  D[0] = a + 2.0 * qx * qx;
+  D[1] = 2.0 * qw * qz + 2.0 * qx * qy;
+  D[2] = -2.0 * qw * qy + 2.0 * qx * qz;
+  D[3] = -2.0 * qw * qz + 2.0 * qy * qx;
+  D[4] = a + 2.0 * qy * qy;
+  D[5] = 2.0 * qw * qx + 2.0 * qy * qz;
+  D[6] = 2.0 * qw * qy + 2.0 * qz * qx;
+  D[7] = -2.0 * qw * qx + 2.0 * qz * qy;
+  D[8] = a + 2.0 * qz * qz;
+  double O[9];
+  for (int i = 0; i < 3; ++i)
+    for (int j = 0; j < 3; ++j) O[3 * i + j] = D[3 * i] * R[j] + D[3 * i + 1] * R[3 + j] + D[3 * i + 2] * R[6 + j];
+  for (int i = 0; i < 9; ++i) R[i] = O[i];
+}
+
 struct Chol2Shared {
   int bad, ok;
   double zz;
 };
 
-template <int MAXSLOT, int ROLE, bool SPLIT>
+__device__ __forceinline__ void c2_help_post(unsigned* hsync, unsigned seq, unsigned accept) {
+  __hip_atomic_store(hsync, ((seq & 0x7fffffffu) << 1) | accept, __ATOMIC_RELAXED, __HIP_MEMORY_SCOPE_AGENT);
+}
+__device__ __forceinline__ double c2_load_sys_f64(const double* p) {
+  return __longlong_as_double((long long)__hip_atomic_load(reinterpret_cast<const unsigned long long*>(p), __ATOMIC_RELAXED,
+                                                           __HIP_MEMORY_SCOPE_SYSTEM));
+}
+
+template <bool SPLIT>
+__device__ __forceinline__ void chol2_helper(double* lds, Chol2Shared& sh) {
+  typedef const Chol2Job __attribute__((address_space(4))) Chol2JobK;
+  typedef const PlaneSolve __attribute__((address_space(4))) PlaneSolveK;
+  typedef const char __attribute__((address_space(4))) KernargByte;
+  PlaneSolveK& pq = *(PlaneSolveK*)((KernargByte*)__builtin_amdgcn_kernarg_segment_ptr() + C2_PS_KERNARG_OFFSET);
+  Chol2JobK& jq = *(Chol2JobK*)__builtin_amdgcn_kernarg_segment_ptr();
+  const int h = (int)blockIdx.x - (SPLIT ? 3 : 2);
+  const int tid = threadIdx.x, wv = tid >> 6, ln = tid & 63;
+  const int n = jq.n;
+  const int nfull = pq.n_full > n ? pq.n_full : n;
+  const int r0 = pq.help_row[h], r1 = pq.help_row[h + 1];
+  const int rend = r1 + C2_HELP_OVERLAP < nfull ? r1 + C2_HELP_OVERLAP : nfull;
+  const int nloc = rend - r0;
+  double* dxs = lds;
+  int* offs = reinterpret_cast<int*>(lds + C2_HELP_NMAX);
+  dbl2_t* Lr = reinterpret_cast<dbl2_t*>(lds + C2_HELP_HDR);
+  if (tid == 0) {
+    int o = 0;
+    for (int j = 0; j < nloc; ++j) {
+      offs[j] = o;
+      o += c2_help_row_pairs(r0 + j, n);
+    }
+  }
+  auto mine = [&](int id) { return id >= r0 && id < r1; };
+  int id = -1, id2 = -1, sid = -1, f0 = -1;
+  double pre[12], pre2[8], sp[3];
+  const int nc = pq.n_clones;
+  if (tid < nc) {
+    id = pq.clone_id[tid];
+    if (mine(id)) {
+      for (int k = 0; k < 9; ++k) pre[k] = pq.clone_R[9 * tid + k];
+      for (int k = 0; k < 3; ++k) pre[9 + k] = pq.clone_p[3 * tid + k];
+    }
+  } else if (tid == nc) {
+    id = pq.calib_id;
+    id2 = pq.intr_id;
+    if (mine(id))
+      for (int k = 0; k < 12; ++k) pre[k] = pq.cal[k];
+    if (mine(id2))
+      for (int k = 0; k < 8; ++k) pre2[k] = pq.cal[12 + k];
+  } else if (tid <= nc + pq.n_planes) {
+    id = pq.plane_sid[tid - nc - 1];
+    if (mine(id))
+      for (int k = 0; k < 3; ++k) pre[k] = pq.cp[3 * (tid - nc - 1) + k];
+  }
+  if (tid < pq.n_slam) {
+    sid = pq.slam_id[tid];
+    if (mine(sid))
+      for (int k = 0; k < 3; ++k) sp[k] = pq.slam_p[3 * tid + k];
+  }
+  if (h == 0 && tid < pq.n_feat_local) f0 = pq.feat_list[tid];
+  __syncthreads();
+  for (int j = wv; j < nloc; j += C2_WAVES) {
+    const int row = r0 + j;
+    const int lastc = row < n ? row : n - 1;
+    const int np = c2_help_row_pairs(row, n);
+    const dbl2_t* lrow = reinterpret_cast<const dbl2_t*>(pq.L0 + (size_t)row * pq.ld0);
+    dbl2_t* dst = Lr + offs[j];
+    for (int q = ln; q < np; q += 64) {
+      dbl2_t v = lrow[q];
+      if (2 * q + 1 > lastc) v[1] = 0.0;
+      dst[q] = v;
+    }
+  }
+  if (tid == 0) {
+    const unsigned want = pq.seq & 0x7fffffffu;
+    int spins = 0;
+    unsigned v = 0u;
+    bool timed_out = false;
+    while (((v = __hip_atomic_load(pq.hsync, __ATOMIC_RELAXED, __HIP_MEMORY_SCOPE_AGENT)) >> 1) != want) {
+      __builtin_amdgcn_s_sleep(2);
+      if (++spins > (1 << 19)) {
+        timed_out = true;
+        break;
+      }
+    }
+    if (timed_out && jq.flag) atomicOr(jq.flag, 2);
+    sh.ok = (!timed_out && (v & 1u)) ? 1 : 0;
+  }
+  __syncthreads();
+  if (!sh.ok) return;
+  dbl2_t yp[3];
+#pragma unroll
+  for (int k = 0; k < 3; ++k) {
+    const int c0 = 2 * (ln + 64 * k);
+    yp[k][0] = c2_load_sys_f64(pq.hy + c0);
+    yp[k][1] = c2_load_sys_f64(pq.hy + c0 + 1);
+  }
+#pragma unroll
+  for (int k = 0; k < 3; ++k) {
+    const int c0 = 2 * (ln + 64 * k);
+    yp[k][0] = c0 < n ? yp[k][0] : 0.0;
+    yp[k][1] = c0 + 1 < n ? yp[k][1] : 0.0;
+  }
+  for (int tb = 0; C2_WAVES * tb < nloc; tb += 16) {
+    double part[16];
+#pragma unroll
+    for (int jj = 0; jj < 16; ++jj) {
+      const int j = wv + C2_WAVES * (tb + jj);
+      double sa = 0.0;
+      if (j < nloc) {
+        const int np = c2_help_row_pairs(r0 + j, n);
+        const dbl2_t* lrow = Lr + offs[j];
+#pragma unroll
+        for (int k = 0; k < 3; ++k) {
+          const int q = ln + 64 * k;
+          if (64 * k < np) {
+            const dbl2_t v = q < np ? lrow[q] : dbl2_t{0.0, 0.0};
+            sa = fma(v[0], yp[k][0], sa);
+            sa = fma(v[1], yp[k][1], sa);
+          }
+        }
+      }
+      part[jj] = sa;
+    }
+    const double tot = wave_transpose_reduce<16>(part);
+    const int j = wv + C2_WAVES * (tb + (ln >> 2));
+    if ((ln & 3) == 0 && j < nloc) dxs[r0 + j] = tot;
+  }
+  __syncthreads();
+  for (int i = r0 + tid; i < r1; i += C2_WAVES * 64) {
+    pq.dx_out[i] = dxs[i];
+    pq.dx_last[i] = dxs[i];
+  }
+  if (h == 0) {
+    if (tid == 0) *pq.cur ^= 1;
+    if (tid == 1 && pq.cond) pq.cond[1] = pq.seq_plane;
+    if (f0 >= 0) pq.feat_used[f0] = 1;
+    for (int i = tid + C2_WAVES * 64; i < pq.n_feat_local; i += C2_WAVES * 64) pq.feat_used[pq.feat_list[i]] = 1;
+  }
+  if (tid < nc) {
+    if (mine(id)) {
+      c2_rot_update(pre, dxs + id);
+      for (int k = 0; k < 9; ++k) pq.clone_R[9 * tid + k] = pre[k];
+      for (int k = 0; k < 3; ++k) pq.clone_p[3 * tid + k] = pre[9 + k] + dxs[id + 3 + k];
+    }
+  } else if (tid == nc) {
+    if (mine(id)) {
+      c2_rot_update(pre, dxs + id);
+      for (int k = 0; k < 9; ++k) pq.cal[k] = pre[k];
+      for (int k = 0; k < 3; ++k) pq.cal[9 + k] = pre[9 + k] + dxs[id + 3 + k];
+    }
+    if (mine(id2))
+      for (int k = 0; k < 8; ++k) pq.cal[12 + k] = pre2[k] + dxs[id2 + k];
+  } else if (tid <= nc + pq.n_planes) {
+    if (mine(id))
+      for (int k = 0; k < 3; ++k) pq.cp[3 * (tid - nc - 1) + k] = pre[k] + dxs[id + k];
+  }
+  if (mine(sid))
+    for (int k = 0; k < 3; ++k) pq.slam_p[3 * tid + k] = sp[k] + dxs[sid + k];
+  for (int q = tid + C2_WAVES * 64; q < pq.n_slam; q += C2_WAVES * 64) {
+    const int s2 = pq.slam_id[q];
+    if (mine(s2))
+      for (int k = 0; k < 3; ++k) pq.slam_p[3 * q + k] += dxs[s2 + k];
+  }
+}
+
+static constexpr int C2_CT_SLOTS = 96;
+static constexpr int C2_CT_STRIDE = 13;
+static constexpr int C2_CT_INTR = C2_CT_SLOTS * C2_CT_STRIDE;
+static constexpr int C2_CT_FEAT = C2_CT_INTR + 8;
+static constexpr int C2_CT_DOUBLES = C2_CT_FEAT + C2_WAVES * 64 / 2;
+static_assert((size_t)(chol2_lds_doubles(18) + C2_CT_DOUBLES) * sizeof(double) <= 160 * 1024, "LDS of the largest plane update");
+__device__ __forceinline__ double* c2_ctab(const Chol2Lds& S) { return reinterpret_cast<double*>(S.cnt) + 8; }
+__device__ __forceinline__ void c2_ctab_prefetch(double* ct) {
+  typedef const PlaneSolve __attribute__((address_space(4))) PlaneSolveK;
+  typedef const char __attribute__((address_space(4))) KernargByte;
+  PlaneSolveK& pq = *(PlaneSolveK*)((KernargByte*)__builtin_amdgcn_kernarg_segment_ptr() + C2_PS_KERNARG_OFFSET);
+  const int tid = threadIdx.x, nc = pq.n_clones;
+  if (nc + pq.n_planes + 1 <= C2_CT_SLOTS) {
+    double* e = ct + C2_CT_STRIDE * tid;
+    if (tid < nc) {
+      for (int k = 0; k < 9; ++k) e[k] = pq.clone_R[9 * tid + k];
+      for (int k = 0; k < 3; ++k) e[9 + k] = pq.clone_p[3 * tid + k];
+      *reinterpret_cast<int*>(e + 12) = pq.clone_id[tid];
+    } else if (tid == nc) {
+      if (pq.calib_id >= 0 || pq.intr_id >= 0) {
+        for (int k = 0; k < 12; ++k) e[k] = pq.cal[k];
+        for (int k = 0; k < 8; ++k) ct[C2_CT_INTR + k] = pq.cal[12 + k];
+      }
+    } else if (tid <= nc + pq.n_planes) {
+      const int pl = tid - nc - 1;
+      for (int k = 0; k < 3; ++k) e[k] = pq.cp[3 * pl + k];
+      *reinterpret_cast<int*>(e + 12) = pq.plane_sid[pl];
+    }
+  }
+  if (tid < pq.n_feat_local) reinterpret_cast<int*>(ct + C2_CT_FEAT)[tid] = pq.feat_list[tid];
+}
+
+template <int MAXSLOT, int ROLE, bool SPLIT, int TAIL>
 __device__ __forceinline__ void chol2_body(const Chol2Job& J0_, const PlaneSolve& ps, double* lds, Chol2Shared& sh, const int joff) {
+  constexpr bool HELP = TAIL == 1, PRE = TAIL == 2;
   typedef const Chol2Job __attribute__((address_space(4))) Chol2JobK;
   typedef const char __attribute__((address_space(4))) KernargByte;
   Chol2JobK& Jf = *(Chol2JobK*)((KernargByte*)__builtin_amdgcn_kernarg_segment_ptr() + joff);
@@ -843,6 +1067,8 @@
   const Chol2Lds S = chol2_carve(lds, nt);
   constexpr int NS = ROLE == 1 ? MAXSLOT : 1;
   if (Jf.skip_cond && Jf.skip_cond[0] != 0 && Jf.skip_cond[0] == Jf.skip_cond[1]) return;
+  if constexpr (PRE)
+    if (Jf.mode == 1 && blockIdx.x == 0) c2_ctab_prefetch(c2_ctab(S));
   double4_t tile[NS];
   int ti[NS], tj[NS];
   int bad = 0;
@@ -1022,7 +1248,11 @@
     }
   }
   __syncthreads();
-  if (!sh_ok) return;
+  if (!sh_ok) {
+    if constexpr (HELP)
+      if (tid == 0 && part != 1) c2_help_post(pq.hsync, pq.seq, 0u);
+    return;
+  }
   M1_STAMP(1);
 
   const int ntn = (n + 15) >> 4;
@@ -1065,9 +1295,21 @@
     if (tid == 0) {
       if (jq.flag) atomicOr(jq.flag, 2);
       pq.res_out[1] = 0.0;
+      if constexpr (HELP) c2_help_post(pq.hsync, pq.seq, 0u);
     }
     return;
   }
+  if constexpr (HELP) {
+    if constexpr (ROLE == 0) {
+      if (wave == 0) {
+        for (int q = lane; 2 * q < n; q += 64)
+          c2_store_through_sys(pq.hy + 2 * q, dbl2_t{S.ybuf[2 * q], 2 * q + 1 < n ? S.ybuf[2 * q + 1] : 0.0});
+        asm volatile("s_waitcnt vmcnt(0)" ::: "memory");
+        if (lane == 0) c2_help_post(pq.hsync, pq.seq, 1u);
+      }
+    }
+    M1_STAMP(3);
+  } else {
   {
     const int wv = tid >> 6, ln = tid & 63;
     dbl2_t yp[3];
@@ -1129,7 +1371,13 @@
     pq.dx_last[i] = dxs[i];
   }
   if (tid == 0) *pq.cur ^= 1;
-  for (int i = tid; i < pq.n_feat_local; i += C2_WAVES * 64) pq.feat_used[pq.feat_list[i]] = 1;
+  double* ct = c2_ctab(S);
+  if constexpr (PRE) {
+    if (tid < pq.n_feat_local) pq.feat_used[reinterpret_cast<const int*>(ct + C2_CT_FEAT)[tid]] = 1;
+    for (int i = tid + C2_WAVES * 64; i < pq.n_feat_local; i += C2_WAVES * 64) pq.feat_used[pq.feat_list[i]] = 1;
+  } else {
+    for (int i = tid; i < pq.n_feat_local; i += C2_WAVES * 64) pq.feat_used[pq.feat_list[i]] = 1;
+  }
   auto rot_update = [&](double* R, const double* dth) {
     double qx = 0.5 * dth[0], qy = 0.5 * dth[1], qz = 0.5 * dth[2], qw = 1.0;
     const double nn = 1.0 / sqrt(qx * qx + qy * qy + qz * qz + qw * qw);
@@ -1153,7 +1401,28 @@
       for (int j = 0; j < 3; ++j) O[3 * i + j] = D[3 * i] * R[j] + D[3 * i + 1] * R[3 + j] + D[3 * i + 2] * R[6 + j];
     for (int i = 0; i < 9; ++i) R[i] = O[i];
   };
-  if (tid < pq.n_clones) {
+  if (PRE && pq.n_clones + pq.n_planes + 1 <= C2_CT_SLOTS) {
+    double* e = ct + C2_CT_STRIDE * tid;
+    if (tid < pq.n_clones) {
+      const int id = *reinterpret_cast<const int*>(e + 12);
+      rot_update(e, dxs + id);
+      for (int k = 0; k < 9; ++k) pq.clone_R[9 * tid + k] = e[k];
+      for (int k = 0; k < 3; ++k) pq.clone_p[3 * tid + k] = e[9 + k] + dxs[id + 3 + k];
+    } else if (tid == pq.n_clones) {
+      if (pq.calib_id >= 0) {
+        rot_update(e, dxs + pq.calib_id);
+        for (int k = 0; k < 9; ++k) pq.cal[k] = e[k];
+        for (int k = 0; k < 3; ++k) pq.cal[9 + k] = e[9 + k] + dxs[pq.calib_id + 3 + k];
+      }
+      if (pq.intr_id >= 0)
+        for (int k = 0; k < 8; ++k) pq.cal[12 + k] = ct[C2_CT_INTR + k] + dxs[pq.intr_id + k];
+    } else if (tid <= pq.n_clones + pq.n_planes) {
+      const int pl = tid - pq.n_clones - 1;
+      const int sid = *reinterpret_cast<const int*>(e + 12);
+      if (sid >= 0)
+        for (int k = 0; k < 3; ++k) pq.cp[3 * pl + k] = e[k] + dxs[sid + k];
+    }
+  } else if (tid < pq.n_clones) {
     const int id = pq.clone_id[tid];
     rot_update(pq.clone_R + 9 * tid, dxs + id);
     for (int k = 0; k < 3; ++k) pq.clone_p[3 * tid + k] += dxs[id + 3 + k];
@@ -1171,9 +1440,11 @@
   }
   for (int q = tid; q < pq.n_slam; q += C2_WAVES * 64)
     for (int k = 0; k < 3; ++k) pq.slam_p[3 * q + k] += dxs[pq.slam_id[q] + k];
+  }
   M1_STAMP(4);
   if (pq.cond) {
-    if (tid == 0) pq.cond[1] = pq.seq_plane;
+    if constexpr (!HELP)
+      if (tid == 0) pq.cond[1] = pq.seq_plane;
     if (pq.emit) {
       if constexpr (ROLE == 1) {
         sfor<MAXSLOT>([&](auto sc) {
@@ -1192,15 +1463,21 @@
   }
 }
 
-template <int MAXSLOT, bool SPLIT>
+template <int MAXSLOT, bool SPLIT, int TAIL>
 __global__ __launch_bounds__(C2_WAVES * 64) void k_chol2(const Chol2Job J0, const Chol2Job J1, const PlaneSolve ps) {
   extern __shared__ __attribute__((aligned(16))) double lds[];
   __shared__ Chol2Shared sh;
+  if constexpr (TAIL == 1) {
+    if (blockIdx.x >= (SPLIT ? 3u : 2u)) {
+      chol2_helper<SPLIT>(lds, sh);
+      return;
+    }
+  }
   const Chol2Job& J = blockIdx.x == 1 ? J1 : J0;
   const int wave = __builtin_amdgcn_readfirstlane((int)threadIdx.x >> 6);
   const int joff = blockIdx.x == 1 ? (int)sizeof(Chol2Job) : 0;
-  if (wave < C2_EW) chol2_body<MAXSLOT, 0, SPLIT>(J, ps, lds, sh, joff);
-  else chol2_body<MAXSLOT, 1, SPLIT>(J, ps, lds, sh, joff);
+  if (wave < C2_EW) chol2_body<MAXSLOT, 0, SPLIT, TAIL>(J, ps, lds, sh, joff);
+  else chol2_body<MAXSLOT, 1, SPLIT, TAIL>(J, ps, lds, sh, joff);
 }
 
 __global__ __launch_bounds__(256) void k_max_diag(const double* __restrict__ A, int n, int ld, double* __restrict__ out) {
@@ -1262,48 +1539,75 @@
     if (nt1 > nt) nt = nt1;
   }
   const int slots = (tiles + C2_TW - 1) / C2_TW;
-  const size_t shmem = (size_t)chol2_lds_doubles(nt) * sizeof(double);
+  size_t shmem = (size_t)chol2_lds_doubles(nt) * sizeof(double);
+  int nh = (ps && j0->mode == 1) ? ps->n_help : 0;
+  if (nh < 0 || nh > C2_MAX_HELP) return hipErrorInvalidValue;
+  if (nh > 0) {
+    if (!j1 || !ps->hy || !ps->hsync || !ps->L0) return hipErrorInvalidValue;
+    const int n = j0->n, nfull = ps->n_full > n ? ps->n_full : n;
+    size_t need = 0;
+    if (c2_help_fits(n, nfull, ps->n_clones, ps->n_planes, nh, ps->help_row, &need)) {
+      if (need > shmem) shmem = need;
+    } else {
+      nh = 0;
+    }
+  }
+  const bool pre = ps && j0->mode == 1 && nh == 0;
+  if (pre) shmem += (size_t)C2_CT_DOUBLES * sizeof(double);
+  if (shmem > 160 * 1024) return hipErrorInvalidValue;
   Chol2Job dummy = *j0;
   PlaneSolve psd = PlaneSolve();
   const Chol2Job& b = j1 ? *j1 : dummy;
-  const PlaneSolve& p = ps ? *ps : psd;
-  const dim3 grid(j0->split_h > 0 ? 3 : (j1 ? 2 : 1)), block(C2_WAVES * 64);
+  if (ps) psd = *ps;
+  psd.n_help = nh;
+  const PlaneSolve& p = psd;
+  const dim3 grid((j0->split_h > 0 ? 3 : (j1 ? 2 : 1)) + nh), block(C2_WAVES * 64);
   static unsigned long long attr_mask = 0;
+#define C2_FOR_EACH_INSTANCE(X) X(10, false) X(15, false) X(17, false) X(20, false) X(22, false) X(13, true) X(16, true) X(22, true)
   if (ovp_lds_attr_needed(&attr_mask)) {
-    (void)hipFuncSetAttribute((const void*)k_chol2<10, false>, hipFuncAttributeMaxDynamicSharedMemorySize, 160 * 1024);
-    (void)hipFuncSetAttribute((const void*)k_chol2<15, false>, hipFuncAttributeMaxDynamicSharedMemorySize, 160 * 1024);
-    (void)hipFuncSetAttribute((const void*)k_chol2<17, false>, hipFuncAttributeMaxDynamicSharedMemorySize, 160 * 1024);
-    (void)hipFuncSetAttribute((const void*)k_chol2<20, false>, hipFuncAttributeMaxDynamicSharedMemorySize, 160 * 1024);
-    (void)hipFuncSetAttribute((const void*)k_chol2<22, false>, hipFuncAttributeMaxDynamicSharedMemorySize, 160 * 1024);
-    (void)hipFuncSetAttribute((const void*)k_chol2<13, true>, hipFuncAttributeMaxDynamicSharedMemorySize, 160 * 1024);
-    (void)hipFuncSetAttribute((const void*)k_chol2<16, true>, hipFuncAttributeMaxDynamicSharedMemorySize, 160 * 1024);
-    (void)hipFuncSetAttribute((const void*)k_chol2<22, true>, hipFuncAttributeMaxDynamicSharedMemorySize, 160 * 1024);
+#define C2_SET_ATTR(MS, SP)                                                                                                        \
+  (void)hipFuncSetAttribute((const void*)k_chol2<MS, SP, 0>, hipFuncAttributeMaxDynamicSharedMemorySize, 160 * 1024);              \
+  (void)hipFuncSetAttribute((const void*)k_chol2<MS, SP, 1>, hipFuncAttributeMaxDynamicSharedMemorySize, 160 * 1024);              \
+  (void)hipFuncSetAttribute((const void*)k_chol2<MS, SP, 2>, hipFuncAttributeMaxDynamicSharedMemorySize, 160 * 1024);
+    C2_FOR_EACH_INSTANCE(C2_SET_ATTR)
+#undef C2_SET_ATTR
     (void)hipGetLastError();
     ovp_lds_attr_done(&attr_mask);
   }
+#undef C2_FOR_EACH_INSTANCE
+#define C2_LAUNCH(MS, SP)                                                                      \
+  do {                                                                                         \
+    if (nh > 0)                                                                                \
+      hipLaunchKernelGGL((k_chol2<MS, SP, 1>), grid, block, shmem, stream, *j0, b, p);         \
+    else if (pre)                                                                              \
+      hipLaunchKernelGGL((k_chol2<MS, SP, 2>), grid, block, shmem, stream, *j0, b, p);         \
+    else                                                                                       \
+      hipLaunchKernelGGL((k_chol2<MS, SP, 0>), grid, block, shmem, stream, *j0, b, p);         \
+  } while (0)
   if (j0->split_h > 0) {
     if (slots <= 13)
-      hipLaunchKernelGGL((k_chol2<13, true>), grid, block, shmem, stream, *j0, b, p);
+      C2_LAUNCH(13, true);
     else if (slots <= 16)
-      hipLaunchKernelGGL((k_chol2<16, true>), grid, block, shmem, stream, *j0, b, p);
+      C2_LAUNCH(16, true);
     else if (slots <= 22)
-      hipLaunchKernelGGL((k_chol2<22, true>), grid, block, shmem, stream, *j0, b, p);
+      C2_LAUNCH(22, true);
     else
       return hipErrorInvalidValue;
     return hipGetLastError();
   }
   if (slots <= 10)
-    hipLaunchKernelGGL((k_chol2<10, false>), grid, block, shmem, stream, *j0, b, p);
+    C2_LAUNCH(10, false);
   else if (slots <= 15)
-    hipLaunchKernelGGL((k_chol2<15, false>), grid, block, shmem, stream, *j0, b, p);
+    C2_LAUNCH(15, false);
   else if (slots <= 17)
-    hipLaunchKernelGGL((k_chol2<17, false>), grid, block, shmem, stream, *j0, b, p);
+    C2_LAUNCH(17, false);
   else if (slots <= 20)
-    hipLaunchKernelGGL((k_chol2<20, false>), grid, block, shmem, stream, *j0, b, p);
+    C2_LAUNCH(20, false);
   else if (slots <= 22)
-    hipLaunchKernelGGL((k_chol2<22, false>), grid, block, shmem, stream, *j0, b, p);
+    C2_LAUNCH(22, false);
   else
     return hipErrorInvalidValue;
+#undef C2_LAUNCH
   return hipGetLastError();
 }
 }
diff --git a/ov_plane_amd/csrc/ovp_api_ctx.hip b/ov_plane_amd/csrc/ovp_api_ctx.hip
--- a/ov_plane_amd/csrc/ovp_api_ctx.hip
+++ b/ov_plane_amd/csrc/ovp_api_ctx.hip
@@ -208,7 +208,7 @@
   void* dev[] = {c->P, c->P_tmp, c->Ab, c->L, c->W1, c->T, c->Lt, c->Y, c->res_block, c->ticket, c->uvn, c->tri_ok, c->state_block, c->batch_block,
                  c->chi2_table, c->G, c->Bscr, c->rec, c->gramS, c->gramR, c->Dinv, c->Ltp, c->part, c->idbuf, c->smallbuf, c->Hd, c->Acc,
                  c->bcc, c->resd, c->pl_slam_i, c->pl_slam_d, c->sub_ids, c->sub_buf, c->pl_Tbuf, c->pl_crow, c->pl_dxlast,
-                 c->pl_cur, c->pl_perm, c->pl_range_done, c->pl_used, c->pl_dstage, c->pl_xbuf, c->pl_xy, c->pl_xflag, c->pl_Asum,
+                 c->pl_cur, c->pl_perm, c->pl_range_done, c->pl_used, c->pl_dstage, c->pl_xbuf, c->pl_xy, c->pl_xflag, c->pl_hy, c->pl_Asum,
                  c->pl_U, c->pl_sub_tab, c->Lkeep, c->slam_res, c->slam_hscr, c->dinit_buf, c->boost, c->boost_vec,
                  c->gen_cal, c->gen_buf, c->pl_gen_dev};
   for (void* p : dev)
@@ -707,6 +707,11 @@
     memcpy(host, &c->pl_hres_cap, sizeof(size_t));
     return (long)sizeof(size_t);
   }
+  else if (!strcmp(name, "clone_R")) { src = c->clone_R; bytes = (size_t)9 * c->fp.n_clones * sizeof(double); if (!src) return OVP_E_STATE; }
+  else if (!strcmp(name, "clone_p")) { src = c->clone_p; bytes = (size_t)3 * c->fp.n_clones * sizeof(double); if (!src) return OVP_E_STATE; }
+  else if (!strcmp(name, "pl_cp")) { src = c->pl_last_cp; bytes = (size_t)3 * c->pl_last_np * sizeof(double); if (!src) return OVP_E_STATE; }
+  else if (!strcmp(name, "pl_slam_p")) { src = c->pl_last_slam_p; bytes = (size_t)3 * c->pl_last_nslam * sizeof(double); if (!src || !bytes) return OVP_E_STATE; }
+  else if (!strcmp(name, "pl_cur")) { src = c->pl_cur; bytes = sizeof(int); if (!src) return OVP_E_STATE; }
   else if (!strcmp(name, "cal")) { src = c->cal; bytes = 20 * sizeof(double); if (!src) return OVP_E_STATE; }
   else if (!strcmp(name, "gen_cal")) { src = c->gen_cal; bytes = (size_t)20 * c->gen_ncams * sizeof(double); if (!src) return OVP_E_STATE; }
   else if (!strcmp(name, "dinit_planes")) {
diff --git a/ov_plane_amd/csrc/ovp_api_plane.hip b/ov_plane_amd/csrc/ovp_api_plane.hip
--- a/ov_plane_amd/csrc/ovp_api_plane.hip
+++ b/ov_plane_amd/csrc/ovp_api_plane.hip
@@ -155,6 +155,26 @@
   return 0;
 }
 
+static int plane_dx_helpers(int nk, int n_full, int n_clones, int n_planes, int* rows) {
+  using namespace ovp;
+  if (n_full < nk) n_full = nk;
+  if (n_full > C2_HELP_NMAX || n_full < 1) return 0;
+  size_t total = 0;
+  for (int r = 0; r < n_full; ++r) total += (size_t)c2_help_row_pairs(r, nk);
+  for (int H = 1; H <= C2_MAX_HELP; ++H) {
+    int r = 0;
+    size_t acc = 0;
+    rows[0] = 0;
+    for (int h = 0; h < H; ++h) {
+      const size_t upto = total * (size_t)(h + 1) / (size_t)H;
+      while (r < n_full && (acc < upto || h == H - 1)) acc += (size_t)c2_help_row_pairs(r++, nk);
+      rows[h + 1] = r;
+    }
+    if (c2_help_fits(nk, n_full, n_clones, n_planes, H, rows, nullptr)) return H;
+  }
+  return 0;
+}
+
 int plane2_buffers(ovp_ctx* c, int NP, size_t stage_bytes, size_t res_bytes) {
   const int ld = c->ld;
   if (!c->pl_Tbuf) {
@@ -167,8 +187,9 @@
     HIPCHK(hipMemset(c->pl_range_done, 0, 16));
     HIPCHK(dalloc(&c->pl_xbuf, (size_t)9 * 18 * 256));
     HIPCHK(dalloc(&c->pl_xy, (size_t)c->n_max + 32));
-    HIPCHK(hipMalloc((void**)&c->pl_xflag, sizeof(unsigned) * 64));
-    HIPCHK(hipMemset(c->pl_xflag, 0, sizeof(unsigned) * 64));
+    HIPCHK(hipMalloc((void**)&c->pl_xflag, sizeof(unsigned) * ovp::C2_XFLAG_WORDS));
+    HIPCHK(hipMemset(c->pl_xflag, 0, sizeof(unsigned) * ovp::C2_XFLAG_WORDS));
+    HIPCHK(dalloc(&c->pl_hy, (size_t)3 * 128));
   }
   if (NP > c->pl2_cap) {
     if (c->pl_perm) hipFree(c->pl_perm);
@@ -709,6 +730,10 @@
   double* d_cpfej = dd + 3 * NP;
   double* d_slam_p = dd + 6 * NP;
   double* d_slam_pfej = dd + 6 * NP + 3 * n_slam;
+  c->pl_last_cp = d_cp;
+  c->pl_last_np = NP;
+  c->pl_last_slam_p = d_slam_p;
+  c->pl_last_nslam = n_slam;
   ovp::PlaneGenParams gp0;
   ovp::PlaneGenCols gcols;
   memset(&gp0, 0, sizeof(gp0));
@@ -772,6 +797,8 @@
   const double white_c = 1.0 / o->sigma_constraint;
   double noise_scale = OVP_PLANE_NOISE_KAPPA;
   if (const char* ns_env = getenv("OVP_PL_NOISE_SCALE")) noise_scale = atof(ns_env);
+  const char* dxi_env = getenv("OVP_C2_DX_INLINE");
+  const bool dx_inline = dxi_env && atoi(dxi_env) != 0;
   for (int jn = 0; jn < NJ; ++jn) {
     const PlaneJobH& j = jobs[jn];
     const int nk = c->pl_sub_active ? c->pl_nl[j.pl] : n;
@@ -892,7 +919,7 @@
       j0.xseq = ps.seq;
       ps.xzz = c->pl_xy;
       ps.xy = c->pl_xy + 16;
-      ps.xsync = c->pl_xflag + 32;
+      ps.xsync = c->pl_xflag + ovp::C2_XFLAG_XSYNC;
     }
     ps.thr = j.thr;
     ps.rows_live = j.rows_live;
@@ -931,6 +958,11 @@
     ps.n_slam = n_slam;
     ps.slam_id = d_sidx;
     ps.slam_p = d_slam_p;
+    if (!dx_inline) {
+      ps.n_help = plane_dx_helpers(nk, n, fp.n_clones, NP, ps.help_row);
+      ps.hy = c->pl_hy;
+      ps.hsync = c->pl_xflag + ovp::C2_XFLAG_HSYNC;
+    }
     if (c->pl_ktimer == 1) {
       while ((int)c->pl_ev.size() < 2 * (jn + 1)) {
         hipEvent_t e;
diff --git a/ov_plane_amd/csrc/ovp_ctx.h b/ov_plane_amd/csrc/ovp_ctx.h
--- a/ov_plane_amd/csrc/ovp_ctx.h
+++ b/ov_plane_amd/csrc/ovp_ctx.h
@@ -195,6 +195,8 @@
   unsigned pl_seq = 0;
   int range_lo = -1, range_hi = -1;
   unsigned char* pl_used = nullptr;
+  const double *pl_last_cp = nullptr, *pl_last_slam_p = nullptr;
+  int pl_last_np = 0, pl_last_nslam = 0;
   std::vector<unsigned char> h_pl_used;
   int* h_slot = nullptr;
   int* d_slot = nullptr;
@@ -204,6 +206,7 @@
   size_t io_cap = 0;
   double *pl_xbuf = nullptr, *pl_xy = nullptr;
   unsigned* pl_xflag = nullptr;
+  double* pl_hy = nullptr;
   double *pl_Asum = nullptr, *pl_U = nullptr;
   int pl_U_cap = 0;
   void *pl_sub_tab = nullptr, *pl_sub_htab = nullptr;
```

Result: faster. 806,000, median of 6 (+1.9%).
